# noir-lang/acvm

Hardware: AMD Instinct MI355X
Metric: witnesses solved/sec (whole node) (higher is better)
Workload: dtype u256 (8x u32 limbs, BN254-Fr Montgomery); 1 GPU; 10000-gate arithmetic-only ACIR, batch 2^20 witnesses over 1 GPU(s); opcodes=10000, global_batch=1048576, instances_per_gpu=1048576, tile_instances=131072, levels=41, not_solved_rank0_all_steps=68, algorithmic_bytes_per_witness=1025376, brillig_opcodes_inlined=0, parallelism=instances sharded x1, no collectives

## Files before the change

acvm_amd/__init__.py:

```python
import ctypes as C
import functools
import os

from . import acir

_HERE = os.path.dirname(os.path.abspath(__file__))
LIB_PATH = os.environ.get("ACVM_AMD_LIB") or os.path.join(_HERE, "libacvm_amd.so")

STATUS_SOLVED, STATUS_IN_PROGRESS, STATUS_FAILURE, STATUS_REQUIRES_FOREIGN_CALL = 0, 1, 2, 3
(ERR_NONE, ERR_MISSING_ASSIGNMENT, ERR_TOO_MANY_UNKNOWNS, ERR_UNSUPPORTED_BLACKBOX, ERR_UNSATISFIED, ERR_INDEX_OOB,
 ERR_BLACKBOX_FAILED, ERR_BRILLIG_FAILED, ERR_PANIC, ERR_DEVICE_LIMIT) = range(10)
LIMIT_BRILLIG_STEPS, LIMIT_BRILLIG_CALL_DEPTH, LIMIT_BRILLIG_MEMORY, LIMIT_DEVICE_MEMORY = 1, 2, 3, 4
ENC_BE32, ENC_LE32, ENC_MONT256_LE = 0, 1, 2
ENC_U8, ENC_U16, ENC_U32, ENC_U64, ENC_U128 = 16, 17, 18, 19, 20
LAYOUT_INSTANCE_MAJOR, LAYOUT_WITNESS_MAJOR = 0, 1
LAYOUT_BROADCAST = 16

ABI_SYMBOLS = [
    "acvm_last_error", "acvm_abi_version", "acvm_device_count", "acvm_set_device", "acvm_device_synchronize",
    "acvm_device_arch", "acvm_selftest", "acvm_debug_grumpkin", "acvm_debug_secp", "acvm_circuit_from_bytes", "acvm_circuit_free", "acvm_circuit_num_opcodes",
    "acvm_circuit_num_witnesses", "acvm_circuit_plan_stats", "acvm_batch_new", "acvm_batch_free", "acvm_batch_set_initial_witness",
    "acvm_batch_set_initial_witness_device", "acvm_batch_solve", "acvm_batch_solve_then_import", "acvm_batch_reset", "acvm_batch_set_instances", "acvm_batch_set_force_slow_path",
    "acvm_batch_results", "acvm_batch_witness", "acvm_batch_witness_map", "acvm_batch_stats",
    "acvm_batch_set_profiling", "acvm_batch_pending_foreign_call", "acvm_batch_pending_foreign_call_inputs",
    "acvm_batch_resolve_foreign_call", "acvm_circuit_assert_message", "acvm_circuit_witness_set", "acvm_batch_error_string",
    "acvm_batch_extract_witnesses", "acvm_batch_digest", "acvm_witness_map_decode", "acvm_witness_map_encode", "acvm_batch_witness_map_bytes",
    "acvm_device_malloc", "acvm_device_free", "acvm_device_upload", "acvm_batch_solve_opcode", "acvm_bb_stubbed", "acvm_bb_dummy",
    "acvm_new", "acvm_free", "acvm_solve", "acvm_solve_opcode", "acvm_get_status", "acvm_instruction_pointer", "acvm_witness_map", "acvm_finalize",
    "acvm_get_pending_foreign_call", "acvm_pending_foreign_call_inputs", "acvm_resolve_pending_foreign_call",
    "acvm_multi_new", "acvm_multi_free", "acvm_multi_num_groups", "acvm_multi_solve", "acvm_multi_results", "acvm_multi_num_witnesses",
    "acvm_multi_witness_map", "acvm_multi_locate", "acvm_debug_modmul_rate", "acvm_debug_secp_rate", "acvm_batch_new_ex", "acvm_circuit_plan_stats_ex",
    "acvm_tuning_set", "acvm_tuning_get", "acvm_tuning_key",
    "acvm_device_release_tables", "acvm_circuit_opcode_kinds", "acvm_batch_error_expression", "acvm_debug_stream_rate", "acvm_node_new", "acvm_node_free", "acvm_node_tile_instances", "acvm_node_num_devices", "acvm_node_solve", "acvm_node_stats",
    "acvm_debug_cpulist", "acvm_debug_device_locality", "acvm_debug_plan_fingerprint", "acvm_circuit_plans_built", "acvm_circuit_check_schedule", "acvm_batch_digest_blake2s",
    "acvm_batch_export_device", "acvm_device_download", "acvm_debug_fr", "acvm_debug_inverse_batch", "acvm_debug_inverse_batch_shared",
    "acvm_batch_import_device", "acvm_batch_solve_then_import_ex",
    "acvm_batch_import_device_parts", "acvm_debug_import_list_copies",
    "acvm_batch_import_device_masked", "acvm_batch_set_initial_witness_masked", "acvm_debug_import_missing",
    "acvm_debug_table_info", "acvm_debug_table_read", "acvm_debug_batch_tables",
    "acvm_batch_outcomes_device", "acvm_batch_export_device_list", "acvm_debug_export_h2d_bytes", "acvm_debug_select",
    "acvm_node_solve_device", "acvm_debug_node_io_bytes",
    "acvm_batch_foreign_call_sites", "acvm_batch_foreign_call_inputs_device", "acvm_batch_resolve_foreign_calls_device", "acvm_debug_foreign_call_stats",
    "acvm_batch_resolve_foreign_calls_device_rows",
    "acvm_node_set_foreign_call_handler", "acvm_node_foreign_stats",
    "acvm_batch_import_device_records", "acvm_batch_set_initial_witness_records", "acvm_node_solve_records",
    "acvm_batch_export_device_records", "acvm_batch_witness_records",
]


class AcvmError(RuntimeError):
    pass


class ExpressionHead(C.Structure):
    _fields_ = [("n_mul", C.c_uint32), ("n_lin", C.c_uint32), ("opcode_index", C.c_uint32), ("q_c", C.c_uint8 * 32)]


class ExportDesc(C.Structure):
    _fields_ = [("encoding", C.c_uint32), ("layout", C.c_uint32), ("first", C.c_uint32), ("n", C.c_uint32), ("witnesses", C.POINTER(C.c_uint32)),
                ("n_witnesses", C.c_uint32), ("stride", C.c_uint64)]


class OutcomesDesc(C.Structure):
    _fields_ = [("first", C.c_uint32), ("n", C.c_uint32), ("d_status", C.c_void_p), ("d_err", C.c_void_p), ("d_opcode_index", C.c_void_p),
                ("select_mask", C.c_uint32), ("d_selected", C.c_void_p)]


class ImportDesc(C.Structure):
    _fields_ = [("encoding", C.c_uint32), ("layout", C.c_uint32), ("columns", C.POINTER(C.c_uint32)), ("n_columns", C.c_uint32), ("stride", C.c_uint64)]


class ImportPart(C.Structure):
    _fields_ = [("d_values", C.c_void_p), ("encoding", C.c_uint32), ("layout", C.c_uint32), ("positions", C.POINTER(C.c_uint32)),
                ("columns", C.POINTER(C.c_uint32)), ("n", C.c_uint32), ("n_columns", C.c_uint32), ("stride", C.c_uint64)]


class RecordField(C.Structure):
    _fields_ = [("position", C.c_uint32), ("encoding", C.c_uint32), ("offset", C.c_uint64)]

# ... 297 lines not shown
    def as_dict(self):
        return {f: (list(getattr(self, f)) if f.startswith("class_") or f == "n_stream_launches" else getattr(self, f)) for f, _ in self._fields_}


_lib = None


def lib():
    global _lib
    if _lib is not None:
        return _lib
    if not os.path.exists(LIB_PATH):
        raise AcvmError(f"{LIB_PATH} is missing: build it with `python -m acvm_amd.build` (no CPU fallback exists)")
    L = C.CDLL(LIB_PATH)
    L.acvm_last_error.restype = C.c_char_p
    L.acvm_device_arch.argtypes = [C.c_char_p, C.c_size_t]
    L.acvm_selftest.argtypes = [C.c_uint32, C.c_uint64]
    L.acvm_debug_grumpkin.argtypes = [C.c_uint32, C.c_uint32, C.c_char_p, C.c_uint32, C.c_char_p]
    if hasattr(L, "acvm_debug_secp"):
        L.acvm_debug_secp.argtypes = [C.c_uint32, C.c_uint32, C.c_char_p, C.c_uint32, C.c_char_p]
    L.acvm_circuit_from_bytes.restype = C.c_void_p
    L.acvm_circuit_from_bytes.argtypes = [C.c_char_p, C.c_size_t]
    L.acvm_circuit_free.argtypes = [C.c_void_p]
    L.acvm_circuit_num_opcodes.restype = C.c_uint32
    L.acvm_circuit_num_opcodes.argtypes = [C.c_void_p]
    L.acvm_circuit_num_witnesses.restype = C.c_uint32
    L.acvm_circuit_num_witnesses.argtypes = [C.c_void_p]
    L.acvm_circuit_plan_stats.argtypes = [C.c_void_p, C.c_void_p, C.c_uint32, C.POINTER(Stats)]
    L.acvm_circuit_plan_stats_ex.argtypes = [C.c_void_p, C.c_void_p, C.c_uint32, C.c_uint32, C.c_void_p, C.c_uint32, C.POINTER(Stats)]
    L.acvm_debug_plan_fingerprint.argtypes = [C.c_void_p, C.c_void_p, C.c_uint32, C.c_uint32, C.c_void_p, C.c_uint32, C.POINTER(C.c_uint64), C.c_uint32]
    L.acvm_circuit_plans_built.restype = C.c_uint64
    L.acvm_circuit_plans_built.argtypes = [C.c_void_p]
    L.acvm_circuit_check_schedule.argtypes = [C.c_void_p, C.c_void_p, C.c_uint32, C.c_uint32, C.c_void_p, C.c_uint32, C.c_uint32, C.c_uint32, C.POINTER(C.c_uint64), C.c_char_p, C.c_size_t]
    L.acvm_batch_new.restype = C.c_void_p
    L.acvm_batch_new.argtypes = [C.c_void_p, C.c_void_p, C.c_uint32, C.c_void_p, C.c_uint32]
    L.acvm_batch_new_ex.restype = C.c_void_p
    L.acvm_batch_new_ex.argtypes = [C.c_void_p, C.c_void_p, C.c_uint32, C.c_void_p, C.c_uint32, C.c_uint32, C.c_void_p, C.c_uint32]
    L.acvm_batch_free.argtypes = [C.c_void_p]
    L.acvm_batch_set_initial_witness.argtypes = [C.c_void_p, C.c_void_p]
    L.acvm_batch_set_initial_witness_device.argtypes = [C.c_void_p, C.c_void_p]
    L.acvm_batch_solve.argtypes = [C.c_void_p]
    L.acvm_batch_solve_then_import.argtypes = [C.c_void_p, C.c_void_p]
    L.acvm_batch_reset.argtypes = [C.c_void_p]
    L.acvm_batch_set_instances.argtypes = [C.c_void_p, C.c_uint32]
    L.acvm_batch_set_force_slow_path.argtypes = [C.c_void_p, C.c_int]
    L.acvm_batch_set_profiling.argtypes = [C.c_void_p, C.c_int]
    L.acvm_batch_results.argtypes = [C.c_void_p, C.c_void_p]
    L.acvm_batch_witness.argtypes = [C.c_void_p, C.c_uint32, C.c_void_p, C.c_void_p]
    L.acvm_batch_witness_map.argtypes = [C.c_void_p, C.c_uint32, C.c_uint32, C.c_void_p, C.c_void_p]
    L.acvm_batch_stats.argtypes = [C.c_void_p, C.POINTER(Stats)]
    L.acvm_batch_pending_foreign_call.argtypes = [C.c_void_p, C.c_uint32, C.POINTER(ForeignCallInfo)]
    L.acvm_batch_pending_foreign_call_inputs.argtypes = [C.c_void_p, C.c_uint32, C.c_void_p, C.c_void_p]
    L.acvm_batch_resolve_foreign_call.argtypes = [C.c_void_p, C.c_uint32, C.c_uint32, C.c_char_p, C.c_void_p, C.c_char_p]
    L.acvm_circuit_assert_message.argtypes = [C.c_void_p, C.c_uint32, C.c_uint32, C.c_char_p, C.c_size_t]
    L.acvm_circuit_witness_set.argtypes = [C.c_void_p, C.c_int, C.c_void_p, C.c_uint32]
    L.acvm_batch_error_string.argtypes = [C.c_void_p, C.c_void_p, C.c_uint32, C.c_char_p, C.c_size_t]
    L.acvm_batch_extract_witnesses.argtypes = [C.c_void_p, C.c_void_p, C.c_uint32, C.c_uint32, C.c_uint32, C.c_void_p]
    L.acvm_batch_digest.argtypes = [C.c_void_p, C.c_uint32, C.c_uint32, C.c_void_p]
    L.acvm_batch_digest_blake2s.argtypes = [C.c_void_p, C.c_uint32, C.c_uint32, C.c_void_p]
    for f in (L.acvm_witness_map_decode, L.acvm_witness_map_encode, L.acvm_batch_witness_map_bytes):
        f.restype = C.c_longlong
    L.acvm_witness_map_decode.argtypes = [C.c_char_p, C.c_size_t, C.c_void_p, C.c_void_p, C.c_uint32]
    L.acvm_witness_map_encode.argtypes = [C.c_void_p, C.c_char_p, C.c_uint32, C.c_void_p, C.c_size_t]
    L.acvm_batch_witness_map_bytes.argtypes = [C.c_void_p, C.c_uint32, C.c_void_p, C.c_size_t]
    L.acvm_debug_modmul_rate.argtypes = [C.c_uint32, C.c_uint32, C.POINTER(C.c_double), C.POINTER(C.c_uint64)]
    if hasattr(L, "acvm_debug_fr"):
# ... 252 lines not shown
    _check(lib().acvm_debug_table_read(table, idx.ctypes.data, idx.size, out.ctypes.data))
    return out


SECP_PROBE_WORDS = ((2, 1), (1, 1), (2, 1), (2, 1), (1, 1), (1, 1), (3, 3), (5, 3), (1, 1), (2, 1), (2, 1), (1, 1),
                    (2, 1), (1, 1), (1, 4), (4, 3), (6, 2))


def debug_secp(curve, what, items):
    wi, wo = SECP_PROBE_WORDS[what]
    assert all(len(it) == wi for it in items)
    data = b"".join(int(v).to_bytes(32, "big") for it in items for v in it)
    out = C.create_string_buffer(32 * wo * max(len(items), 1))
    _check(lib().acvm_debug_secp(curve, what, data, len(items), out))
    raw = out.raw
    return [tuple(int.from_bytes(raw[32 * (wo * i + k):32 * (wo * i + k + 1)], "big") for k in range(wo)) for i in range(len(items))]


FR_PROBE_WORDS = ((16, 8), (16, 8), (8, 8), (16, 8), (16, 8), (8, 8), (8, 8), (8, 8), (8, 8), (8, 2), (8, 2), (1, 8), (8, 9), (9, 8), (18, 9), (18, 9), (9, 9),
                  (9, 1), (9, 9), (10, 9), (9, 9), (9, 9), (9, 9), (9, 9), (19, 9), (18, 9), (9, 9), (9, 1), (18, 9), (36, 9), (54, 9), (27, 9), (45, 9), (27, 9),
                  (45, 9), (18, 9), (36, 9), (27, 9))


def debug_fr(what, items, uniform=None):
    import numpy as np
    wi, wo = FR_PROBE_WORDS[what]
    a = np.ascontiguousarray(items, dtype=np.uint32).reshape(-1, wi)
    out = np.zeros((a.shape[0], wo), dtype=np.uint32)
    u = None if uniform is None else np.ascontiguousarray(uniform, dtype=np.uint32).reshape(18)
    _check(lib().acvm_debug_fr(what, a.ctypes.data, a.shape[0], None if u is None else u.ctypes.data, out.ctypes.data))
    return out


def debug_inverse_batch(den, inv_chunk, slot_of=None, inv_share=None):
    import numpy as np
    d = np.ascontiguousarray(den, dtype=np.uint32)
    n_jobs, B = d.shape[0], d.shape[1]
    assert d.shape == (n_jobs, B, 8)
    s = None if slot_of is None else np.ascontiguousarray(slot_of, dtype=np.uint32).reshape(n_jobs)
    inv, ev = np.zeros((n_jobs, B, 8), dtype=np.uint32), np.zeros(B, dtype=np.uint32)
    dc, hc = C.c_uint32(), C.c_uint32()
    if inv_share is None:
        _check(lib().acvm_debug_inverse_batch(d.ctypes.data, n_jobs, B, inv_chunk, None if s is None else s.ctypes.data, inv.ctypes.data, ev.ctypes.data,
                                              C.byref(dc), C.byref(hc)))
    else:
        _check(lib().acvm_debug_inverse_batch_shared(d.ctypes.data, n_jobs, B, inv_chunk, inv_share, None if s is None else s.ctypes.data, inv.ctypes.data,
                                                     ev.ctypes.data, C.byref(dc), C.byref(hc)))
    return inv, ev, dc.value, hc.value


def debug_select(status, select_mask, out=None, want_list=True):
    import numpy as np
    st = np.ascontiguousarray(status, dtype=np.uint8).reshape(-1)
    n = st.shape[0]
    lst = None
    if want_list:
        lst = np.zeros(n, dtype=np.uint32) if out is None else np.ascontiguousarray(out, dtype=np.uint32).reshape(n).copy()
    count = C.c_uint32()
    _check(lib().acvm_debug_select(st.ctypes.data if n else None, n, select_mask, lst.ctypes.data if lst is not None and n else None, C.byref(count)))
    return lst, count.value


def decompress_witness(data: bytes) -> dict:
    n = _check(lib().acvm_witness_map_decode(data, len(data), None, None, 0))
    ids = (C.c_uint32 * max(n, 1))()
    vals = C.create_string_buffer(32 * max(n, 1))
# ... 40 lines not shown
        n = lib().acvm_circuit_assert_message(self._h, acir_index, self.LOCATION_ACIR if brillig_index is None else brillig_index, buf, 4096)
        return None if n < 0 else buf.value.decode()

    def witness_set(self, which: str):
        n = _check(lib().acvm_circuit_witness_set(self._h, self.SETS[which], None, 0))
        arr = (C.c_uint32 * max(n, 1))()
        _check(lib().acvm_circuit_witness_set(self._h, self.SETS[which], arr, n))
        return list(arr[:n])

    def plan_stats(self, initial_ids, fold_digest=False, reuse_slots=False, keep=()) -> dict:
        ids = list(initial_ids)
        arr = (C.c_uint32 * max(len(ids), 1))(*ids)
        keep = list(keep)
        karr = (C.c_uint32 * max(len(keep), 1))(*keep)
        s = Stats()
        _check(lib().acvm_circuit_plan_stats_ex(self._h, arr, len(ids), (1 if fold_digest else 0) | (2 if reuse_slots else 0), karr, len(keep), C.byref(s)))
        return s.as_dict()

    def plans_built(self) -> int:
        return int(lib().acvm_circuit_plans_built(self._h))

    def check_schedule(self, initial_ids, n_instances=4096, fold_digest=False, reuse_slots=False, keep=(), host_solver=False, drop_wait=None) -> dict:
        ids = list(initial_ids)
        arr = (C.c_uint32 * max(len(ids), 1))(*ids)
        keep = list(keep)
        karr = (C.c_uint32 * max(len(keep), 1))(*keep)
        counts = (C.c_uint64 * 8)()
        text = C.create_string_buffer(1 << 14)
        rc = lib().acvm_circuit_check_schedule(self._h, arr, len(ids), (1 if fold_digest else 0) | (2 if reuse_slots else 0) | (0x100 if host_solver else 0),
                                               karr, len(keep), n_instances, 0xFFFFFFFF if drop_wait is None else drop_wait, counts, text, len(text))
        _check(rc)
        return {"ok": rc == 0, "n_launches": counts[0], "n_waits": counts[1], "n_accesses": counts[2], "n_records": counts[3], "n_findings": counts[4],
                "report": text.value.decode()}

    def plan_fingerprint(self, initial_ids, fold_digest=False, reuse_slots=False, keep=(), host_solver=False) -> list:
        ids = list(initial_ids)
        arr = (C.c_uint32 * max(len(ids), 1))(*ids)
        keep = list(keep)
        karr = (C.c_uint32 * max(len(keep), 1))(*keep)
        out = (C.c_uint64 * 128)()
        n = lib().acvm_debug_plan_fingerprint(self._h, arr, len(ids), (1 if fold_digest else 0) | (2 if reuse_slots else 0) | (0x100 if host_solver else 0),
                                              karr, len(keep), out, 128)
        _check(n)
        return list(out[:n])


class NodeOpts(C.Structure):
    _fields_ = [("n_devices", C.c_uint32), ("devices", C.POINTER(C.c_int)), ("tile_instances", C.c_uint32), ("batch_flags", C.c_uint32)]


class NodeStats(C.Structure):
    _fields_ = [("n_devices", C.c_uint32), ("tile_instances", C.c_uint32), ("n_instances", C.c_uint64), ("total_ms", C.c_double),
                ("device", C.c_int * 16), ("async_exact", C.c_uint32 * 16), ("tiles", C.c_uint32 * 16), ("exact_instances", C.c_uint32 * 16),
                ("lane_ms", C.c_double * 16), ("solve_device_ms", C.c_double * 16), ("h2d_wait_ms", C.c_double * 16), ("export_ms", C.c_double * 16),
                ("numa_node", C.c_int * 16), ("n_cpus_pinned", C.c_uint32 * 16), ("first_cpu", C.c_int * 16),
                ("plans_built", C.c_uint32), ("create_ms", C.c_double), ("plan_ms", C.c_double), ("host_rss_bytes", C.c_uint64)]


class Node:

    def __init__(self, circuit: "Circuit", initial_ids, keep=(), devices=None, tile=0, fold_digest=False, reuse_slots=False, solver: "BbSolver" = None):
        self.ids, self.keep = list(initial_ids), list(keep)
        self._solver = solver
        arr = (C.c_uint32 * max(len(self.ids), 1))(*self.ids)
        karr = (C.c_uint32 * max(len(self.keep), 1))(*self.keep)
        opts = NodeOpts()
# ... 620 lines not shown
```

acvm_amd/csrc/batch.cpp:

```cpp
#include <algorithm>
#include <chrono>
#include <cstdio>
#include <cstdlib>
#include <cstring>
#include <map>
#include <memory>
#include <new>
#include <stdexcept>
#include <string>
#include <vector>
#include "batch_internal.hpp"

static thread_local std::string g_last_error;
int set_err(int code, const std::string &msg) {
    g_last_error = msg;
    return code;
}

int stage_reserve(acvm_batch *b, size_t bytes) {
    if (bytes <= b->stage_cap) return 0;
    if (b->d_stage) { hipFree(b->d_stage); b->d_stage = nullptr; b->stage_cap = 0; }
    const size_t cap = std::max<size_t>(bytes + bytes / 4, (size_t)1 << 20);
    HIPCHK(hipMalloc((void **)&b->d_stage, cap));
    b->stage_cap = cap;
    return 0;
}
void clear_fc_store(acvm_batch *b) {
    for (auto &sl : b->fc_slots) {
        if (sl.device_owned) {
            sl.device_owned = false;
            sl.clear_pending = true;
            sl.bounds = FcBounds();
        }
        if (!sl.inst.empty()) { sl.inst.clear(); sl.dirty = true; }
    }
    b->fc_fail_msg.clear();
    b->fc_epoch++;
}

const char *acvm_last_error(void) { return g_last_error.c_str(); }
int acvm_abi_version(void) { return ACVM_AMD_ABI_VERSION; }

int acvm_device_count(void) {
    int n = 0;
// ... 141 lines not shown
    out->n_brillig_inlined = p.n_brillig_inlined;
    out->n_hash_chained = p.n_hash_chained;
    out->n_gate_out_asis = p.n_gate_out_mode[0];
    out->n_gate_out_weak = p.n_gate_out_mode[1];
    out->n_gate_out_canon = p.n_gate_out_mode[2];
    out->max_gate_bound = p.max_gate_bound;
    out->n_byte_planes = p.n_byte_planes;
    out->n_byte_plane_reads = p.n_byte_plane_reads;
    for (uint32_t L = 0; L + 1 < p.level_start.size(); L++) out->n_arith_launches += (p.level_start[L + 1] - p.level_start[L] + 65534) / 65535;
    for (int k = 0; k < 4; k++) out->class_algorithmic_bytes_per_instance[k] = p.cls_algorithmic_bytes[k];
    out->class_algorithmic_bytes_per_instance[CLS_GRUMPKIN] += p.cls_algorithmic_bytes[CLS_PEDERSEN] + p.cls_algorithmic_bytes[CLS_ECDSA] +
                                                               p.cls_algorithmic_bytes[CLS_HOSTBB];
}

int acvm_circuit_plan_stats(const acvm_circuit_t *c, const uint32_t *initial_ids, uint32_t n_initial, acvm_stats_t *out) {
    return acvm_circuit_plan_stats_ex(c, initial_ids, n_initial, 0, nullptr, 0, out);
}
int acvm_circuit_plan_stats_ex(const acvm_circuit_t *c, const uint32_t *initial_ids, uint32_t n_initial, uint32_t flags, const uint32_t *keep_ids,
                               uint32_t n_keep, acvm_stats_t *out) try {
    if (!c || !out || (n_initial && !initial_ids) || (n_keep && !keep_ids)) return set_err(ACVM_E_INVALID, "null argument");
    PlanOpts opts;
    opts.fold_digest = (flags & (ACVM_BATCH_FOLD_DIGEST | ACVM_BATCH_REUSE_SLOTS)) != 0;
    opts.reuse_slots = (flags & ACVM_BATCH_REUSE_SLOTS) != 0;
    opts.keep.assign(keep_ids, keep_ids + n_keep);
    const std::shared_ptr<const Plan> sp = plan_for(c, initial_ids, n_initial, opts);
    const Plan &p = *sp;
    plan_stats(p, out);
    if (!p.unsupported.empty()) return set_err(ACVM_E_UNSUPPORTED, p.unsupported);
    return 0;
} ABI_CATCH

static size_t plan_bytes(const Plan &p) {
    size_t words = p.gate_stream.size() + p.gate_offset.size() + p.prog.size() + p.prog_offset.size() + p.prog_scratch.size() + p.bytecode.size() + p.slot_of.size() + p.kbound.size() +
                   p.unscale_index.size() + p.scaled_ids.size() + p.producer.size() + p.byte_plane_of.size() + p.dyn_offset.size();
    for (int k = 0; k < (int)N_CLS; k++) words += 2 * p.cls_offset[k].size();
    return words * 4 + (p.constants.size() + p.unscale.size()) * sizeof(FrH);
}
static void remember_plan(const acvm_circuit *c, const std::shared_ptr<const Plan> &sp) {
    auto &v = c->recent_plans;
    v.erase(std::remove(v.begin(), v.end(), sp), v.end());
    v.push_back(sp);
    size_t total = 0;
    for (auto &q : v) total += plan_bytes(*q);
    while (v.size() > 1 && (v.size() > 8 || total > (1ull << 30))) { total -= plan_bytes(*v.front()); v.erase(v.begin()); }
}
std::shared_ptr<const Plan> plan_for(const acvm_circuit *c, const uint32_t *initial_ids, uint32_t n_initial, const PlanOpts &opts) {
    PlanKey key;
    key.ids.assign(initial_ids, initial_ids + n_initial);
    if (opts.reuse_slots) key.keep = opts.keep;
    key.host_blackbox = opts.host_blackbox;
    key.fold_digest = opts.fold_digest;
    key.reuse_slots = opts.reuse_slots;
    for (unsigned i = 0; const char *name = tuning_key(i); i++) {
        int64_t v = 0;
        tuning_get(name, &v);
        key.tuning.push_back(v);
    }
    {
        std::lock_guard<std::mutex> g(c->plan_mutex);
        for (auto it = c->plan_cache.begin(); it != c->plan_cache.end();) {
            std::shared_ptr<const Plan> sp = it->second.lock();
            if (!sp) { it = c->plan_cache.erase(it); continue; }
            if (it->first == key) { c->n_plans_shared++; remember_plan(c, sp); return sp; }
            ++it;
        }
    }
    std::shared_ptr<const Plan> sp = std::make_shared<const Plan>(build_plan(*c->c, initial_ids, n_initial, opts));
    std::lock_guard<std::mutex> g(c->plan_mutex);
    c->n_plans_built++;
    c->plan_cache.push_back({std::move(key), sp});
    remember_plan(c, sp);
    return sp;
}
uint64_t acvm_circuit_plans_built(const acvm_circuit_t *c) {
    if (!c) return 0;
    std::lock_guard<std::mutex> g(c->plan_mutex);
    return c->n_plans_built;
}

int acvm_circuit_check_schedule(const acvm_circuit_t *c, const uint32_t *initial_ids, uint32_t n_initial, uint32_t flags, const uint32_t *keep_ids, uint32_t n_keep,
                                uint32_t n_instances, uint32_t drop_wait, uint64_t *counts, char *report, size_t report_len) try {
    if (!c || (n_initial && !initial_ids) || (n_keep && !keep_ids)) return set_err(ACVM_E_INVALID, "null argument");
    PlanOpts opts;
    opts.fold_digest = (flags & (ACVM_BATCH_FOLD_DIGEST | ACVM_BATCH_REUSE_SLOTS)) != 0;
    opts.reuse_slots = (flags & ACVM_BATCH_REUSE_SLOTS) != 0;
    opts.host_blackbox = (flags & 0x100u) != 0;
    opts.keep.assign(keep_ids, keep_ids + n_keep);
    const std::shared_ptr<const Plan> sp = plan_for(c, initial_ids, n_initial, opts);
    if (!sp->unsupported.empty()) return set_err(ACVM_E_UNSUPPORTED, sp->unsupported);
    const LaunchLayout lay = layout_launches(*sp, ((uint64_t)n_instances + 63) / 64 * 64);
    const LevelSchedule sched = level_schedule(*sp, lay);
    const ScheduleReport rep = check_level_schedule(*sp, lay, sched, drop_wait);
    if (counts) { counts[0] = rep.n_launches; counts[1] = rep.n_waits; counts[2] = rep.n_accesses; counts[3] = rep.n_records; counts[4] = rep.n_findings; }
    if (report && report_len) snprintf(report, report_len, "%s", rep.text.c_str());
    return rep.ok ? 0 : 1;
} ABI_CATCH

int acvm_debug_plan_fingerprint(const acvm_circuit_t *c, const uint32_t *initial_ids, uint32_t n_initial, uint32_t flags, const uint32_t *keep_ids,
                                uint32_t n_keep, uint64_t *out, uint32_t cap) try {
    if (!c || !out || (n_initial && !initial_ids) || (n_keep && !keep_ids)) return set_err(ACVM_E_INVALID, "null argument");
    PlanOpts opts;
    opts.fold_digest = (flags & (ACVM_BATCH_FOLD_DIGEST | ACVM_BATCH_REUSE_SLOTS)) != 0;
    opts.reuse_slots = (flags & ACVM_BATCH_REUSE_SLOTS) != 0;
    opts.host_blackbox = (flags & 0x100u) != 0;
    opts.keep.assign(keep_ids, keep_ids + n_keep);
    const Plan p = build_plan(*c->c, initial_ids, n_initial, opts);
    if (!p.unsupported.empty()) return set_err(ACVM_E_UNSUPPORTED, p.unsupported);
    std::vector<uint64_t> fp;
    auto fnv = [](const void *data, size_t bytes, uint64_t h = 0xcbf29ce484222325ull) {
        const uint8_t *b = (const uint8_t *)data;
        for (size_t i = 0; i < bytes; i++) { h ^= b[i]; h *= 0x100000001b3ull; }
        return h;
    };
    auto vec = [&](const std::vector<uint32_t> &v) { fp.push_back(fnv(v.data(), v.size() * 4) ^ (uint64_t)v.size() << 40); };
    vec(p.gate_stream); vec(p.gate_offset); vec(p.level_start); vec(p.dyn_offset); vec(p.dyn_level_start); vec(p.level_needs_inverse);
    for (int q = 0; q < N_HEAVY_LANES; q++) { vec(p.level_needs_heavy[q]); vec(p.inv_needs_heavy[q]); vec(p.lane_needs_main[q]); for (int q2 = 0; q2 < N_HEAVY_LANES; q2++) vec(p.lane_needs_lane[q][q2]); }
    vec(p.prog); vec(p.prog_offset); vec(p.prog_scratch); vec(p.slot_of); vec(p.kbound); vec(p.scaled_ids); vec(p.unscale_index); vec(p.bytecode); vec(p.producer); vec(p.byte_plane_of);
    fp.push_back(fnv(p.constants.data(), p.constants.size() * sizeof(FrH)));
    fp.push_back(fnv(p.unscale.data(), p.unscale.size() * sizeof(FrH)));
    fp.push_back(fnv(p.prog_class.data(), p.prog_class.size()));
    for (int k = 0; k < (int)N_CLS; k++) {
        vec(p.cls_level_start[k]);
        std::vector<uint32_t> sorted;
        for (size_t L = 0; L + 1 < p.cls_level_start[k].size(); L++) {
            std::vector<std::pair<uint32_t, uint32_t>> lv;
            for (uint32_t r = p.cls_level_start[k][L]; r < p.cls_level_start[k][L + 1]; r++) lv.push_back({p.cls_offset[k][r], p.cls_scratch[k][r]});
            std::sort(lv.begin(), lv.end());
            for (auto &x : lv) { sorted.push_back(x.first); sorted.push_back(x.second); }
        }
        vec(sorted);
    }
    const uint32_t scal[] = {p.n_witnesses, p.n_opcodes, p.n_levels, p.n_slots, p.mem_cells, p.n_inverse_slots, p.n_digest_segments, p.truncated_at, p.n_byte_planes};
    fp.push_back(fnv(scal, sizeof scal));
    for (size_t i = 0; i < fp.size() && i < cap; i++) out[i] = fp[i];
    return (int)fp.size();
} ABI_CATCH


static int batch_init(acvm_batch *b) {
    HIPCHK(hipGetDevice(&b->device));
    hipDeviceProp_t prop;
    HIPCHK(hipGetDeviceProperties(&prop, b->device));
    if (strncmp(prop.gcnArchName, "gfx950", 6) != 0)
        return set_err(ACVM_E_DEVICE, std::string("device is ") + prop.gcnArchName + ", this library is built for gfx950 only");
    HIPCHK(hipStreamCreateWithFlags(&b->stream, hipStreamNonBlocking));
    HIPCHK(hipStreamCreateWithFlags(&b->stream_dyn, hipStreamNonBlocking));
    HIPCHK(hipStreamCreateWithFlags(&b->stream_heavy, hipStreamNonBlocking));
    HIPCHK(hipStreamCreateWithFlags(&b->stream_heavy2, hipStreamNonBlocking));
    HIPCHK(hipStreamCreateWithFlags(&b->stream_heavy3, hipStreamNonBlocking));
    HIPCHK(hipStreamCreateWithFlags(&b->stream_digest, hipStreamNonBlocking));
    HIPCHK(hipEventCreate(&b->ev_start));
    HIPCHK(hipEventCreate(&b->ev_end));
    const Plan &p = b->plan();
    size_t w_bytes = (size_t)(b->reuse() ? p.n_slots : p.n_witnesses) * 2 * b->Bp * sizeof(uint4);
    HIPCHK(hipMalloc((void **)&b->d_W, w_bytes ? w_bytes : 16));
    if (int rc = upload(&b->d_gate_stream, p.gate_stream)) return rc;
    if (int rc = upload(&b->d_gate_offset, p.gate_offset)) return rc;
    std::vector<uint32_t> consts(p.constants.size() * 8);
    for (size_t i = 0; i < p.constants.size(); i++) {
        const FrH d = frh::to_device_form(p.constants[i]);
        memcpy(&consts[8 * i], d.l, 32);
    }
    if (int rc = upload(&b->d_consts, consts)) return rc;
    if (!p.scaled_ids.empty()) {
        std::vector<uint32_t> uc(p.unscale.size() * 8);
        for (size_t i = 0; i < p.unscale.size(); i++) {
            const FrH d = frh::to_device_form(p.unscale[i]);
            memcpy(&uc[8 * i], d.l, 32);
        }
        if (int rc = upload(&b->d_unscale_consts, uc)) return rc;
        for (size_t i = 0; i < p.unscale.size(); i++) {
            uint64_t c[4];
            frh::to_canonical(p.unscale[i], c);
            memcpy(&uc[8 * i], c, 32);
        }
        if (int rc = upload(&b->d_unscale_plain, uc)) return rc;
        if (int rc = upload(&b->d_unscale_index, p.unscale_index)) return rc;
        if (int rc = upload(&b->d_scaled_ids, p.scaled_ids)) return rc;
    }
    if (int rc = upload(&b->d_prog, p.prog)) return rc;
    if (int rc = upload(&b->d_prog_offset, p.prog_offset)) return rc;
    if (int rc = upload(&b->d_bytecode, p.bytecode)) return rc;
    if (int rc = upload(&b->d_init_ids, p.initial_ids)) return rc;
    if (p.n_byte_planes) {
        b->plane_of_input.resize(p.initial_ids.size());
        for (size_t i = 0; i < p.initial_ids.size(); i++) b->plane_of_input[i] = p.byte_plane_of[p.initial_ids[i]];
        if (int rc = upload(&b->d_byte_plane_of, p.byte_plane_of)) return rc;
        if (int rc = upload(&b->d_byte_plane_of_input, b->plane_of_input)) return rc;
        HIPCHK(hipMalloc((void **)&b->d_byte_plane, (size_t)p.n_byte_planes * b->Bp * 4));
        HIPCHK(hipMemsetAsync(b->d_byte_plane, 0, (size_t)p.n_byte_planes * b->Bp * 4, b->stream));
// ... 192 lines not shown
```

acvm_amd/csrc/batch.hpp:

```cpp
#pragma once
#include "../../include/acvm_amd.h"
#include "foreign_plan.hpp"
#include "import_plan.hpp"
#include "kernels.hpp"
#include "plan.hpp"
#include "schedule.hpp"
#include <map>
#include <memory>
#include <mutex>
#include <string>
#include <vector>

using namespace acvm;

int set_err(int code, const std::string &msg);
#define HIPCHK(expr)                                                                                      \
    do {                                                                                                  \
        hipError_t _e = (expr);                                                                           \
        if (_e != hipSuccess)                                                                             \
            return set_err(ACVM_E_DEVICE, std::string(#expr) + ": " + hipGetErrorString(_e));             \
    } while (0)

#define ABI_CATCH                                                                                          \
    catch (const std::bad_alloc &) { return set_err(ACVM_E_NOMEM, "out of host memory"); }                 \
// ... 22 lines not shown
    uint8_t *d_digests = nullptr;
    uint64_t *h2d = nullptr;
};

struct PlanKey {
    std::vector<uint32_t> ids, keep;
    bool host_blackbox = false, fold_digest = false, reuse_slots = false;
    std::vector<int64_t> tuning;
    bool operator==(const PlanKey &o) const {
        return ids == o.ids && keep == o.keep && host_blackbox == o.host_blackbox && fold_digest == o.fold_digest && reuse_slots == o.reuse_slots && tuning == o.tuning;
    }
};
struct acvm_circuit {
    std::unique_ptr<Circuit> c;
    mutable std::mutex plan_mutex;
    mutable std::vector<std::pair<PlanKey, std::weak_ptr<const Plan>>> plan_cache;
    mutable std::vector<std::shared_ptr<const Plan>> recent_plans;
    mutable uint64_t n_plans_built = 0, n_plans_shared = 0;
};
std::shared_ptr<const Plan> plan_for(const acvm_circuit *c, const uint32_t *initial_ids, uint32_t n_initial, const acvm::PlanOpts &opts);

struct acvm_batch {
    std::shared_ptr<const Plan> plan_ref;
    const Plan &plan() const { return *plan_ref; }
    LaunchLayout layout;
    LevelSchedule schedule;
    uint32_t B = 0;
    uint32_t capacity = 0;
    uint64_t Bp = 0;
    int device = 0;
    hipStream_t stream = nullptr;
    uint4 *d_W = nullptr, *d_Mem = nullptr;
    uint32_t *d_gate_stream = nullptr, *d_gate_offset = nullptr, *d_consts = nullptr;
    uint32_t *d_prog = nullptr, *d_prog_offset = nullptr, *d_bytecode = nullptr, *d_init_ids = nullptr, *d_producer = nullptr;
    uint32_t *d_dyn_offset = nullptr, *d_slow_start = nullptr;
    uint8_t *d_prog_class = nullptr;
    uint32_t *d_cls_offset[N_CLS] = {nullptr, nullptr, nullptr, nullptr, nullptr, nullptr, nullptr};
    uint32_t *d_cls_scratch_off[N_CLS] = {nullptr, nullptr, nullptr, nullptr, nullptr, nullptr, nullptr};
    uint32_t *d_cls_scratch[N_CLS] = {nullptr, nullptr, nullptr, nullptr, nullptr, nullptr, nullptr};
    DeviceProgram dp{};
    uint32_t *d_event = nullptr;
    uint32_t *d_event_base = nullptr;
    uint32_t *h_flag_count = nullptr;
    bool events_fresh = false;
    std::vector<uint32_t> h_event;
    bool events_clean = false;
    std::vector<uint32_t> slow_ids, slow_start;
    std::vector<int32_t> slow_index;
    std::vector<SlowResult> slow_res;
    uint32_t *d_slow_ids = nullptr, *d_assigned = nullptr;
    SlowResult *d_slow_res = nullptr;
    uint32_t slow_cap = 0, n_words = 0;
    bool inputs_set = false, solved = false, force_slow = false, profiling = false;
    hipEvent_t ev_start = nullptr, ev_end = nullptr;
    std::vector<hipEvent_t> ev_pool;
    double solve_device_ms = 0, arith_kernel_ms = 0, dyn_kernel_ms = 0, slow_path_ms = 0;
    double cls_kernel_ms[N_CLS] = {0, 0, 0, 0, 0, 0, 0};
    hipStream_t stream_dyn = nullptr, stream_heavy = nullptr, stream_heavy2 = nullptr, stream_heavy3 = nullptr, stream_digest = nullptr;
    PlanOpts opts;
    uint4 *d_leaves = nullptr;
    uint32_t *d_fp_g = nullptr, *d_fp_gs = nullptr, *d_fp_h = nullptr, *d_fp_hgen = nullptr;
    DigestTables fp{};
    uint32_t *d_slot_of = nullptr;
    uint4 *d_Wx = nullptr, *d_Memx = nullptr;
    uint32_t *d_init_rows = nullptr, *d_ids_x = nullptr;
    uint32_t *d_byte_plane_of = nullptr, *d_byte_plane_of_input = nullptr, *d_byte_plane = nullptr;
// ... 73 lines not shown
    std::vector<FcSlot> fc_slots;
    FcStoreSlot *d_fc_store = nullptr;
    uint32_t *d_fc_pend_desc = nullptr;
    uint4 *d_fc_pend_vals = nullptr;
    uint32_t fc_pend_desc_words = 0, fc_pend_vals_cap = 0, fc_lanes_cap = 0;
    std::vector<uint32_t> h_pend_desc, h_pend_vals;
    bool pend_host_valid = false;
    uint64_t n_fc_h2d_bytes = 0, n_fc_d2h_bytes = 0;
    hipEvent_t ev_fc[2] = {nullptr, nullptr};
    uint64_t fc_epoch = 1, fc_rows_key[4] = {0, 0, 0, 0};
    std::vector<uint32_t> fc_rows_host;
    uint32_t *d_fc_rows = nullptr;
    size_t fc_rows_cap = 0;
    uint8_t *d_fc_mask = nullptr;
    size_t fc_mask_cap = 0;
    bool fc_rows_valid = false, fc_rows_longest_valid = false;
    uint32_t fc_rows_longest = 0;
    double fc_inputs_ms = 0, fc_append_ms = 0;
    uint8_t *d_stage = nullptr;
    size_t stage_cap = 0;
    uint8_t *d_fetch = nullptr;
    bool stepping = false;
    uint32_t *d_br_scratch = nullptr, *d_br_lane = nullptr;
    size_t br_scratch_bytes = 0;
    uint32_t br_lane_cap = 0;
    bool br_retry_active = false;
    uint32_t br_max_regs = 1;
    uint32_t n_brillig_retries = 0;

    ~acvm_batch() {
        hipSetDevice(device);
        for (void *p : {(void *)d_W, (void *)d_Mem, (void *)d_gate_stream, (void *)d_gate_offset, (void *)d_consts, (void *)d_prog,
                        (void *)d_prog_offset, (void *)d_bytecode, (void *)d_init_ids, (void *)d_producer, (void *)d_dyn_offset,
                        (void *)d_slow_start, (void *)d_event_base, (void *)d_slow_ids, (void *)d_assigned, (void *)d_slow_res})
            if (p) hipFree(p);
        if (h_flag_count) hipHostFree(h_flag_count);
        for (int k = 0; k < (int)N_CLS; k++)
            for (void *p : {(void *)d_cls_offset[k], (void *)d_cls_scratch_off[k], (void *)d_cls_scratch[k]})
                if (p) hipFree(p);
        for (auto e : ev_pool) hipEventDestroy(e);
        for (auto e : ev_sync) hipEventDestroy(e);
        for (auto e : ev_heavy) hipEventDestroy(e);
        if (stream_heavy) hipStreamDestroy(stream_heavy);
        if (stream_heavy2) hipStreamDestroy(stream_heavy2);
        if (stream_heavy3) hipStreamDestroy(stream_heavy3);
        if (stream_digest) hipStreamDestroy(stream_digest);
        if (d_prog_class) hipFree(d_prog_class);
        if (d_leaves) hipFree(d_leaves);
        for (void *p : {(void *)d_fp_g, (void *)d_fp_gs, (void *)d_fp_h, (void *)d_fp_hgen})
            if (p) hipFree(p);
        if (d_slot_of) hipFree(d_slot_of);
        for (void *p : {(void *)d_Wx, (void *)d_Memx, (void *)d_init_rows, (void *)d_ids_x, (void *)d_byte_plane_of, (void *)d_byte_plane_of_input, (void *)d_byte_plane})
            if (p) hipFree(p);
        if (d_inv) hipFree(d_inv);
        for (void *p : {(void *)d_unscale_index, (void *)d_unscale_consts, (void *)d_unscale_plain, (void *)d_scaled_ids, (void *)d_unscale_m256})
            if (p) hipFree(p);
        if (d_ped_seed) hipFree(d_ped_seed);
        if (d_stage) hipFree(d_stage);
        if (d_fetch) hipFree(d_fetch);
        if (d_import_lists) hipFree(d_import_lists);
        if (d_missing) hipFree(d_missing);
        if (d_mask_result) hipFree(d_mask_result);
        if (h_mask_result) hipHostFree(h_mask_result);
        if (d_lane_map) hipFree(d_lane_map);
        if (d_record_out_tables) hipFree(d_record_out_tables);
        for (uint8_t *q : d_sink)
            if (q) hipFree(q);
// ... 47 lines not shown
```

acvm_amd/csrc/batch_schedule.cpp:

```cpp
#include <algorithm>
#include <chrono>
#include <cstdio>
#include <cstdlib>
#include <cstring>
#include <map>
#include <memory>
#include <new>
#include <stdexcept>
#include <string>
#include <vector>
#include "batch_internal.hpp"

struct LaunchTimers {
    std::vector<std::pair<hipEvent_t, hipEvent_t>> reg_pairs, dyn_pairs, cls_pairs[N_CLS];
    size_t ev_used = 0;
};

static int enqueue_level_schedule(acvm_batch *b, LaunchTimers *tm) {
    const Plan &p = b->plan();
    auto next_event = [&]() -> hipEvent_t {
        if (tm->ev_used == b->ev_pool.size()) {
            hipEvent_t e;
            hipEventCreate(&e);
            b->ev_pool.push_back(e);
        }
        return b->ev_pool[tm->ev_used++];
    };
    const bool prof = tm != nullptr;
    hipStream_t streams[N_SCHED_STREAMS] = {b->stream, b->stream_dyn, b->stream_heavy, b->stream_heavy2, b->stream_heavy3, b->stream_digest};
    const uint32_t n_sync = 2 * p.n_levels + 1;
    auto event_of = [&](uint32_t id) { return id < n_sync ? b->ev_sync[id] : b->ev_heavy[id - n_sync]; };
    for (const SchedStep &st : b->schedule.steps) {
        hipStream_t s = streams[st.stream];
        if (st.kind == SK_RECORD) { HIPCHK(hipEventRecord(event_of(st.event), s)); continue; }
        if (st.kind == SK_WAIT) { HIPCHK(hipStreamWaitEvent(s, event_of(st.event), 0)); continue; }
        const int k = st.cls;
        const uint32_t *off = b->d_cls_offset[k] + st.first, *soff = b->d_cls_scratch_off[k] + 2 * (size_t)st.first;
        const bool timed = prof && st.op != SO_EVENT_RESET && st.op != SO_TRUNCATE;
        hipEvent_t e0 = nullptr, e1 = nullptr;
        if (timed) { e0 = next_event(); hipEventRecord(e0, s); }
        switch (st.op) {
        case SO_EVENT_RESET:
            if (!b->events_fresh) launch_event_reset(s, b->d_event, b->B);
            b->events_fresh = false;
            break;
        case SO_GATES:
            launch_arith_level(s, b->d_W, b->Bp, b->B, b->d_gate_stream, b->d_gate_offset + st.first, st.count, b->d_consts, b->d_event, b->d_inv);
            break;
        case SO_GATES_LIGHT:
            launch_arith_light_level(s, b->d_W, b->Bp, b->B, b->d_gate_stream, b->d_gate_offset + st.first, st.count, b->d_inv, b->dp,
                                     b->d_cls_offset[CLS_LIGHT] + st.first2, st.count2, b->d_event);
            break;
        case SO_LIGHT: launch_light_level(s, b->d_W, b->Bp, b->B, b->dp, off, st.count, b->d_event); break;
        case SO_LIGHT_SL: launch_light_sl_level(s, b->d_W, b->Bp, b->B, b->dp, off, st.count, b->d_event); break;
        case SO_HASH_COOP: launch_hash_coop_level(s, b->d_W, b->Bp, b->B, b->dp, off, st.count, b->d_event, st.lds_words); break;
        case SO_HASH: launch_hash_level(s, b->d_W, b->Bp, b->B, b->dp, off, soff, st.count, b->d_event, b->d_cls_scratch[k]); break;
        case SO_GRUMPKIN: launch_grumpkin_level(s, b->d_W, b->Bp, b->B, b->dp, off, soff, st.count, b->d_event, b->d_cls_scratch[k]); break;
        case SO_BRILLIG: launch_brillig_level(s, b->d_W, b->Bp, b->B, b->dp, off, soff, st.count, b->d_event, b->d_cls_scratch[k]); break;
        case SO_PEDERSEN: launch_pedersen_level(s, b->d_W, b->Bp, b->B, b->dp, off, st.count, b->d_event, soff, b->d_cls_scratch[k]); break;
        case SO_ECDSA: launch_ecdsa_level(s, b->d_W, b->Bp, b->B, b->dp, off, st.count, b->d_event); break;
        case SO_DIGEST: launch_digest_fold_level(s, b->d_W, b->Bp, b->B, b->dp, off, st.count, b->fp, b->d_leaves); break;
        case SO_HOSTBB:
            for (uint32_t r = 0; r < st.count; r++)
                if (int rc = run_host_blackbox(b, p.prog[p.cls_offset[k][st.first + r] + 1], false, 0)) return rc;
            break;
        case SO_INVERSE:
            launch_inverse_batch(s, b->d_W, b->d_inv, b->Bp, b->B, b->d_gate_stream, b->d_dyn_offset + st.first, st.count, b->d_event, (uint32_t)p.tune.inv_chunk,
                                 inverse_share_clamp(p.tune.inv_share));
            break;
        case SO_TRUNCATE: launch_event_truncate(s, b->d_event, b->B, p.truncated_at); break;
        }
        if (timed) {
            e1 = next_event();
            hipEventRecord(e1, s);
            (st.op == SO_GATES || st.op == SO_GATES_LIGHT ? tm->reg_pairs : st.op == SO_INVERSE ? tm->dyn_pairs : tm->cls_pairs[k]).push_back({e0, e1});
        }
        if (st.op == SO_GATES || st.op == SO_GATES_LIGHT) b->n_launches += (st.count + 65534) / 65535;
        else if (st.op != SO_EVENT_RESET && st.op != SO_TRUNCATE) b->n_launches++;
    }
    return 0;
}

static int ensure_level_events(acvm_batch *b) {
    const size_t n_levels = b->plan().n_levels;
// ... 203 lines not shown
```

acvm_amd/csrc/fr_device.hpp:

```cpp
#pragma once
#include <hip/hip_runtime.h>
#include <stdint.h>

#define FR_HD __host__ __device__

namespace acvm {

struct Fr {
    uint32_t v[8];
};

#define FR_P0 0xf0000001u
#define FR_P1 0x43e1f593u
#define FR_P2 0x79b97091u
#define FR_P3 0x2833e848u
#define FR_P4 0x8181585du
#define FR_P5 0xb85045b6u
#define FR_P6 0xe131a029u
#define FR_P7 0x30644e72u
#define FR_N0INV 0xefffffffu

FR_HD __forceinline__ uint32_t fr_p(int i) {
    constexpr uint32_t P[8] = {FR_P0, FR_P1, FR_P2, FR_P3, FR_P4, FR_P5, FR_P6, FR_P7};
    return P[i];
// ... 290 lines not shown
#pragma unroll
    for (int k = 0; k < 9; k++) {
#pragma unroll
        for (int t = 0; t < N; t++)
#pragma unroll
            for (int i = 0; i <= k; i++) acc += (uint64_t)a[t].v[i] * b[t].v[k - i];
#pragma unroll
        for (int i = 0; i < k; i++) acc += (uint64_t)m[i] * fr_p29(k - i);
        const uint32_t lo = (uint32_t)acc;
        m[k] = (((lo & 1u) << 28) - lo) & M;
        acc += ((uint64_t)m[k] << 28) + m[k];
        acc >>= 29;
    }
#pragma unroll
    for (int k = 9; k < 17; k++) {
#pragma unroll
        for (int t = 0; t < N; t++)
#pragma unroll
            for (int i = k - 8; i < 9; i++) acc += (uint64_t)a[t].v[i] * b[t].v[k - i];
#pragma unroll
        for (int i = k - 8; i < 9; i++) acc += (uint64_t)m[i] * fr_p29(k - i);
        if (ADD) acc += h->v[k - 9];
        r.v[k - 9] = (uint32_t)acc & M;
        acc >>= 29;
    }
    r.v[8] = (uint32_t)acc;
    if (ADD) r.v[8] += h->v[8];
    return r;
}
template <int N>
FR_HD __forceinline__ Fr29 fr29_dot(const Fr29 (&a)[N], const Fr29 (&b)[N]) { return fr29_dot_impl<N, false>(a, b, nullptr); }
template <int N>
FR_HD __forceinline__ Fr29 fr29_dot_add(const Fr29 (&a)[N], const Fr29 (&b)[N], const Fr29 &h) { return fr29_dot_impl<N, true>(a, b, &h); }

#if defined(__HIP_DEVICE_COMPILE__) && !defined(FR_NO_ASM_BLOCKS)
#define FR_ASM_BLOCKS 1
#include "fr_blocks.inc"
#endif
#ifdef FR_BLOCKS_ALL
#undef fr29_mul
FR_HD __forceinline__ Fr29 fr29_mul(const Fr29 &a, const Fr29 &b) {
#if FR_ASM_BLOCKS
    return fr29_mul_blk(a, b);
#else
    return fr29_mul_c(a, b);
#endif
}
#endif
FR_HD __forceinline__ Fr29 fr29_mul_b(const Fr29 &a, const Fr29 &b) {
#if FR_ASM_BLOCKS
    return fr29_mul_blk(a, b);
#else
    return fr29_mul(a, b);
#endif
}
template <int N, unsigned UB>
FR_HD __forceinline__ Fr29 fr29_dot_add_b(const Fr29 (&a)[N], const Fr29 (&b)[N], const Fr29 &h) {
    static_assert(N == 1 || N == 2, "generated forms");
#if FR_ASM_BLOCKS
    if constexpr (N == 1) {
        static_assert(UB <= 1u, "one product");
        if constexpr (UB == 1u) return fr29_dot1_add_blk_u(a[0], b[0], h);
        else return fr29_dot1_add_blk_v(a[0], b[0], h);
    } else {
        static_assert(UB == 0u || UB == 2u || UB == 3u, "a uniform first factor pairs with a uniform second one");
        if constexpr (UB == 0u) return fr29_dot2_add_blk_vv(a[0], b[0], a[1], b[1], h);
// ... 259 lines not shown
```

acvm_amd/csrc/gate_eval.hpp:

```cpp
#pragma once
#include "fr_device.hpp"
#include "gate_record.hpp"

namespace acvm {

FR_HD __forceinline__ void gate_h_room(Fr29 &h, uint32_t &hw, uint32_t weight) {
    if (hw + weight > GATE_H_MAX) {
        h = fr29_weak(fr29_norm(h));
        hw = GATE_H_AFTER_WEAK;
    }
    hw += weight;
}
FR_HD __forceinline__ void gate_h_sub(Fr29 &h, const Fr29 &x, uint32_t klog2) {
    if (klog2 <= 1) {
#pragma unroll
        for (int i = 0; i < 9; i++) h.v[i] += fr_kp29_sub(1, i) - x.v[i];
    } else if (klog2 == 2) {
#pragma unroll
        for (int i = 0; i < 9; i++) h.v[i] += fr_kp29_sub(2, i) - x.v[i];
    } else {
#pragma unroll
        for (int i = 0; i < 9; i++) h.v[i] += fr_kp29_sub(3, i) - x.v[i];
    }
}
FR_HD __forceinline__ Fr29 gate_coef29(GateWords t) {
    Fr c;
#pragma unroll
    for (int i = 0; i < 8; i++) c.v[i] = t[i];
    return fr29_from(c);
}

template <class L>
FR_HD __forceinline__ Fr29 gate_operand(const L &ld, uint32_t slot, const Fr29 &local) {
    if (slot == GATE_LOCAL) {
        Fr29 r = local;
#if defined(__HIP_DEVICE_COMPILE__)
#pragma unroll
        for (int k = 0; k < 9; k++) asm volatile("" : "+v"(r.v[k]));
#endif
        return r;
    }
    return ld.load(slot);
}
FR_HD __forceinline__ GateWords gate_mac_entry(GateWords t0, uint32_t np_mac, uint32_t k) {
    return k < np_mac ? t0 + 10 * k : t0 + 10 * np_mac + 9 * (k - np_mac);
}
template <class L>
FR_HD __forceinline__ Fr29 gate_mac_operand(const L &ld, GateWords c, bool product, const Fr29 &local) {
    if (product) return fr29_mul_b(gate_operand(ld, c[8], local), gate_operand(ld, c[9], local));
    return gate_operand(ld, c[8], local);
}

template <class L>
FR_HD __forceinline__ Fr29 gate_eval(const L &ld, GateWords g, const Fr29 &local) {
    const uint32_t w0 = g[0], w5 = g[5], qc = g[3], kind = w0 & 0xff;
    const uint32_t np_mac = (w0 >> 8) & 0xff, nl_mac = (w0 >> 16) & 0xff, n_mac = np_mac + nl_mac;
    const uint32_t np_pos = w5 & 0xff, np_neg = (w5 >> 8) & 0xff, nl_pos = (w5 >> 16) & 0xff, nl_neg = w5 >> 24;
    const uint32_t sub_k = (w0 >> GATE_SUBK_SHIFT) & 3u;
    Fr29 h;
    uint32_t hw = 0;
    if (qc == GATE_COEF_ZERO) {
#pragma unroll
        for (int i = 0; i < 9; i++) h.v[i] = 0;
    } else {
        h = gate_coef29(ld.constant(qc));
        hw = 16;
    }
    GateWords t0 = g + 6;
    GateWords tp = t0 + 10 * np_mac + 9 * nl_mac;
    GateWords t = tp + 2 * np_pos;
    for (uint32_t i = 0; i < np_neg; i++, t += 2) {
        const Fr29 x = fr29_mul_b(gate_operand(ld, t[0], local), gate_operand(ld, t[1], local));
        gate_h_room(h, hw, 33);
        gate_h_sub(h, x, 1);
    }
    for (uint32_t i = 0; i < nl_pos; i++, t += 1) {
        const Fr29 x = gate_operand(ld, t[0], local);
        gate_h_room(h, hw, 16);
        h = fr29_addl(h, x);
    }
    for (uint32_t i = 0; i < nl_neg; i++, t += 1) {
        const Fr29 x = gate_operand(ld, t[0], local);
        gate_h_room(h, hw, 33);
        gate_h_sub(h, x, sub_k);
    }
    uint32_t im = 0, ip = 0, n_red = 0;
    bool normalised = false;
#define GATE_AFTER_REDUCTION() do { normalised = true; if (++n_red == GATE_REDUCTIONS_PER_WEAK) { h = fr29_weak(h); n_red = 0; } } while (0)
    for (; ip < np_pos && im < n_mac; ip++, im++) {
        GateWords c = gate_mac_entry(t0, np_mac, im);
        const Fr29 l[2] = {gate_operand(ld, tp[2 * ip], local), gate_mac_operand(ld, c, im < np_mac, local)};
        const Fr29 m[2] = {gate_operand(ld, tp[2 * ip + 1], local), gate_coef29(c)};
        h = fr29_dot_add_b<2, 2u>(l, m, h);
        GATE_AFTER_REDUCTION();
    }
    for (; im < n_mac; im += 2) {
        GateWords c0 = gate_mac_entry(t0, np_mac, im);
        if (n_mac - im == 1) {
            const Fr29 l[1] = {gate_mac_operand(ld, c0, im < np_mac, local)}, m[1] = {gate_coef29(c0)};
            h = fr29_dot_add_b<1, 1u>(l, m, h);
        } else {
            GateWords c1 = gate_mac_entry(t0, np_mac, im + 1);
            const Fr29 l[2] = {gate_mac_operand(ld, c0, im < np_mac, local), gate_mac_operand(ld, c1, im + 1 < np_mac, local)};
            const Fr29 m[2] = {gate_coef29(c0), gate_coef29(c1)};
            h = fr29_dot_add_b<2, 3u>(l, m, h);
        }
        GATE_AFTER_REDUCTION();
    }
    for (; ip < np_pos; ip += 2) {
        if (np_pos - ip == 1) {
            const Fr29 l[1] = {gate_operand(ld, tp[2 * ip], local)}, m[1] = {gate_operand(ld, tp[2 * ip + 1], local)};
            h = fr29_dot_add_b<1, 0u>(l, m, h);
        } else {
            const Fr29 l[2] = {gate_operand(ld, tp[2 * ip], local), gate_operand(ld, tp[2 * ip + 2], local)};
            const Fr29 m[2] = {gate_operand(ld, tp[2 * ip + 1], local), gate_operand(ld, tp[2 * ip + 3], local)};
            h = fr29_dot_add_b<2, 0u>(l, m, h);
        }
        GATE_AFTER_REDUCTION();
    }
#undef GATE_AFTER_REDUCTION
    Fr29 acc = normalised ? h : fr29_norm(h);
    if (kind == 2) {
        if (w0 & GATE_PRESUM_WEAK) acc = fr29_weak(acc);
        acc = fr29_mul_b(acc, ld.load_inverse(g[4]));
    }
    const uint32_t mode = kind == 0 ? GATE_OUT_CANON : (w0 >> GATE_OUT_SHIFT) & 3u;
    if (mode != GATE_OUT_ASIS) {
        acc = fr29_weak(acc);
        if (mode == GATE_OUT_CANON) {
            if (ld.any(acc.v[8] >= fr_p29(8))) acc = fr29_csub(acc, 0);
        }
// ... 6 lines not shown
```

acvm_amd/csrc/gate_record.hpp:

```cpp
#pragma once
#include <stdint.h>

#if defined(__HIPCC__)
#define GATE_HD __host__ __device__
#else
#define GATE_HD
#endif

namespace acvm {

#if defined(__HIP_DEVICE_COMPILE__)
typedef const uint32_t __attribute__((address_space(4))) *GateWords;
#define GATE_WORDS(p) ((::acvm::GateWords)(uintptr_t)(p))
#else
typedef const uint32_t *GateWords;
#define GATE_WORDS(p) ((::acvm::GateWords)(p))
#endif

static constexpr uint32_t GATE_LOCAL = 0xFFFFFFFFu;
static constexpr uint32_t GATE_TAIL_FLAG = 1u << 24;
static constexpr uint32_t GATE_SETLOCAL_FLAG = 1u << 25;
static constexpr uint32_t GATE_OUT_SHIFT = 26;
static constexpr uint32_t GATE_OUT_ASIS = 0;
static constexpr uint32_t GATE_OUT_WEAK = 1;
static constexpr uint32_t GATE_OUT_CANON = 2;
static constexpr uint32_t GATE_SUBK_SHIFT = 28;
static constexpr uint32_t GATE_PRESUM_WEAK = 1u << 30;
static constexpr uint32_t GATE_COEF_ZERO = 0xFFFFFFFDu;

static constexpr uint32_t GATE_H_MAX = 111;
static constexpr uint32_t GATE_H_AFTER_WEAK = 17;
static constexpr uint32_t GATE_REDUCTIONS_PER_WEAK = 16;

static constexpr uint32_t GATE_K_CANON = 256, GATE_K_WEAK = 264, GATE_K_ROW_MAX = 1354, GATE_K_INVERSE = 359;
GATE_HD inline uint32_t gate_k_product(uint32_t ka, uint32_t kb) {
    return (uint32_t)(((uint64_t)ka * kb * 1549u + ((1ull << 26) - 1)) >> 26);
}

GATE_HD inline uint32_t gate_record_words(GateWords g) {
    const uint32_t w0 = g[0], w5 = g[5];
    return 6u + 10u * ((w0 >> 8) & 0xff) + 9u * ((w0 >> 16) & 0xff) + 2u * ((w5 & 0xff) + ((w5 >> 8) & 0xff)) + ((w5 >> 16) & 0xff) + (w5 >> 24);
}

}
```

acvm_amd/csrc/kernels.hip:

```cpp
#include "ops_common.hpp"
#include "fr_probe.hpp"
#include "inverse_batch.hpp"
#include "kernels.hpp"
#include "export_encode.hpp"
#include "export_source.hpp"
#include "tuning.hpp"

namespace acvm {

template <bool ALIGNED>
__global__ void __launch_bounds__(256) import_witness_kernel(uint4 *__restrict__ W, uint64_t Bp, uint32_t B,
                                                             const uint8_t *__restrict__ in, const uint32_t *__restrict__ ids,
                                                             uint32_t n_in, const uint32_t *__restrict__ gate, const uint32_t *__restrict__ plane_of_input,
                                                             uint32_t *__restrict__ plane, uint32_t *__restrict__ event_reset) {
    __shared__ uint4 tile[4][2][65];
    __shared__ uint32_t tile_low[4][64];
    if (gate && *gate != 0u) return;
    const uint32_t t = threadIdx.x;
    const uint64_t j0 = (uint64_t)blockIdx.x * 64u;
    const uint32_t k0 = blockIdx.y * 4u;
    {
        const uint32_t ji = t >> 2, kk = t & 3u;
        const uint64_t j = j0 + ji;
        const uint32_t k = k0 + kk;
// ... 231 lines not shown
    __syncthreads();
#pragma unroll
    for (uint32_t step = 0; step < export_tile_steps(T); step++) {
        const ExportTileUnit q = export_tile_unit(T, t, step);
        const uint64_t i = i0 + q.ji;
        const uint32_t k = kb + q.kk;
        if (i >= a.n || k >= a.n_sel) continue;
        const uint64_t at = export_element_index(EXPORT_INSTANCE_MAJOR, a.stride, i, k);
        export_store_nt(a.out + 2 * at + q.half, tile[q.kk][q.half][q.ji]);
        if (a.mask && q.half == 0) a.mask[at] = tile_assigned[q.kk][q.ji];
    }
}
__global__ void __launch_bounds__(256) unscale_slow_kernel(uint4 *__restrict__ W, uint64_t Bp, const uint32_t *__restrict__ slow_ids,
                                                           uint32_t n_slow, const uint32_t *__restrict__ scaled_ids, uint32_t n_scaled,
                                                           const uint32_t *__restrict__ consts, const uint32_t *__restrict__ producer,
                                                           const uint32_t *__restrict__ start_opcode) {
    const uint64_t i = (uint64_t)blockIdx.x * blockDim.x + threadIdx.x;
    if (i >= (uint64_t)n_slow * n_scaled) return;
    const uint32_t k = (uint32_t)(i / n_slow), t = (uint32_t)(i % n_slow);
    const uint64_t j = slow_ids[t];
    const uint32_t w = scaled_ids[k];
    if (producer[w] >= start_opcode[t]) return;
    fr_store(W, w, Bp, j, fr_mul(fr_load(W, w, Bp, j), fr_const(consts, k)));
}

#ifndef ARITH_BLOCK
#define ARITH_BLOCK 256
#endif
#ifndef ARITH_WAVES_MIN
#define ARITH_WAVES_MIN 6
#endif
__global__ void __launch_bounds__(ARITH_BLOCK) __attribute__((amdgpu_waves_per_eu(ARITH_WAVES_MIN, 8)))
arith_level_kernel(uint4 *__restrict__ W, uint64_t Bp, uint32_t B, const uint32_t *__restrict__ gate_stream, const uint32_t *__restrict__ gate_offset,
                   const uint32_t *__restrict__ consts, uint32_t *__restrict__ event, const uint4 *__restrict__ Inv) {
    arith_level_body(W, Bp, B, gate_stream, gate_offset, consts, event, Inv, blockIdx.y);
}

struct InverseDevicePolicy {
    static __device__ __forceinline__ Fr load_den(const uint4 *W, uint32_t row, uint64_t Bp, uint64_t j) { return fr_load(W, row, Bp, j); }
    static __device__ __forceinline__ Fr load_den_last(const uint4 *W, uint32_t row, uint64_t Bp, uint64_t j) { return fr_load_nt(W, row, Bp, j); }
    static __device__ __forceinline__ void park(uint4 *Inv, uint32_t slot, uint64_t Bp, uint64_t j, const Fr &a) { fr_store(Inv, slot, Bp, j, a); }
    static __device__ __forceinline__ Fr parked(const uint4 *Inv, uint32_t slot, uint64_t Bp, uint64_t j) { return fr_load(Inv, slot, Bp, j); }
    static __device__ __forceinline__ void store_inverse(uint4 *Inv, uint32_t slot, uint64_t Bp, uint64_t j, const Fr &a) { fr_store_nt(Inv, slot, Bp, j, a); }
    static __device__ __forceinline__ void flag(uint32_t *event, uint64_t j, uint32_t opcode) { flag_instance(event, j, opcode); }
};
__global__ void __launch_bounds__(64) inverse_batch_kernel(const uint4 *__restrict__ W, uint4 *__restrict__ Inv, uint64_t Bp, uint32_t B,
                                                           const uint32_t *__restrict__ gate_stream, const uint32_t *__restrict__ job_offset,
                                                           uint32_t n_jobs, uint32_t chunk, uint32_t *__restrict__ event) {
    const uint64_t j = (uint64_t)blockIdx.x * 64 + threadIdx.x;
    if (j >= B) return;
    const uint32_t first = blockIdx.y * chunk;
    const uint32_t n = n_jobs - first < chunk ? n_jobs - first : chunk;
    inverse_batch_body<InverseDevicePolicy>(W, Inv, Bp, j, gate_stream, job_offset, first, n, event);
}
template <int G>
__global__ void __launch_bounds__(64 * G) inverse_batch_kernel_shared(const uint4 *__restrict__ W, uint4 *__restrict__ Inv, uint64_t Bp, uint32_t B,
                                                                      const uint32_t *__restrict__ gate_stream, const uint32_t *__restrict__ job_offset,
                                                                      uint32_t n_jobs, uint32_t chunk, uint32_t *__restrict__ event) {
    __shared__ uint32_t rows[(G + 1) * INVERSE_SHARE_ROW_WORDS];
    const uint32_t lane = threadIdx.x & 63u, w = __builtin_amdgcn_readfirstlane(threadIdx.x >> 6);
    const uint64_t j = (uint64_t)blockIdx.x * (64 * G) + threadIdx.x;
    const bool live = j < B;
    const uint32_t first = blockIdx.y * chunk;
    const uint32_t n = n_jobs - first < chunk ? n_jobs - first : chunk;
    Fr29 total = fr29_from(fr_one());
    if (live) total = inverse_batch_forward<InverseDevicePolicy>(W, Inv, Bp, j, gate_stream, job_offset, first, n, event);
    inverse_share_row_store(rows, w, lane, total);
    __syncthreads();
// ... 78 lines not shown
        }
        auto same = [](const Fr29 &p, const Fr29 &q) {
            uint32_t d = 0;
#pragma unroll
            for (int k = 0; k < 9; k++) d |= p.v[k] ^ q.v[k];
            return d == 0;
        };
        if (!same(fr29_mul_b(x, y), fr29_mul(x, y)) || !same(fr29_mul_b(y, x), fr29_mul(y, x))) bad |= 512;
        const Fr29 l1[1] = {x}, m1v[1] = {y}, m1u[1] = {u};
        if (!same(fr29_dot_add_b<1, 0u>(l1, m1v, h), fr29_dot_add<1>(l1, m1v, h))) bad |= 1024;
        if (!same(fr29_dot_add_b<1, 1u>(l1, m1u, h), fr29_dot_add<1>(l1, m1u, h))) bad |= 1024;
        const Fr29 l2[2] = {x, z}, m2vv[2] = {y, x}, m2vu[2] = {y, u}, m2uu[2] = {w, u};
        if (!same(fr29_dot_add_b<2, 0u>(l2, m2vv, h), fr29_dot_add<2>(l2, m2vv, h))) bad |= 2048;
        if (!same(fr29_dot_add_b<2, 2u>(l2, m2vu, h), fr29_dot_add<2>(l2, m2vu, h))) bad |= 2048;
        if (!same(fr29_dot_add_b<2, 3u>(l2, m2uu, h), fr29_dot_add<2>(l2, m2uu, h))) bad |= 2048;
    }
    if (bad) atomicAdd(mismatches, 1u);
}

__global__ void __launch_bounds__(64) fr_probe_kernel(uint32_t what, const uint32_t *__restrict__ in, uint32_t n_items, uint32_t words_in, uint32_t words_out,
                                                      FrProbeUniform un, uint32_t *__restrict__ out) {
    const uint32_t t = blockIdx.x * 64 + threadIdx.x;
    if (t >= n_items) return;
    fr_probe_item(what, in + (size_t)t * words_in, un, out + (size_t)t * words_out);
}
uint32_t fr_probe_words(uint32_t what, bool out) { return out ? fr_probe_words_out(what) : fr_probe_words_in(what); }
void launch_fr_probe(hipStream_t s, uint32_t what, const uint32_t *in, uint32_t n_items, const uint32_t *uniform18, uint32_t *out) {
    if (!n_items || what >= FRP_COUNT) return;
    FrProbeUniform un;
    for (int k = 0; k < 18; k++) un.u[k / 9].v[k % 9] = uniform18 ? uniform18[k] : 0u;
    hipLaunchKernelGGL(fr_probe_kernel, dim3((n_items + 63) / 64), dim3(64), 0, s, what, in, n_items, fr_probe_words_in(what), fr_probe_words_out(what), un, out);
}

__global__ void __launch_bounds__(256) modmul_rate_kernel(uint32_t *__restrict__ out, uint32_t seed, uint32_t iters) {
    Fr29 a, b;
#pragma unroll
    for (int i = 0; i < 9; i++) {
        a.v[i] = ((threadIdx.x + 1) * 2654435761u + seed + i) & 0x1fffffffu;
        b.v[i] = (a.v[i] ^ 0x5bd1e995u) & 0x1fffffffu;
    }
    a.v[8] &= 0xfffffu;
    b.v[8] &= 0xfffffu;
    for (uint32_t i = 0; i < iters; i++) {
        a = fr29_mul(a, b);
        b = fr29_mul(b, a);
    }
    uint32_t s = 0;
#pragma unroll
    for (int i = 0; i < 9; i++) s += a.v[i] ^ b.v[i];
    out[(uint64_t)blockIdx.x * blockDim.x + threadIdx.x] = s;
}
__global__ void __launch_bounds__(256) stream_rate_kernel(const uint4 *__restrict__ a, const uint4 *__restrict__ b, uint4 *__restrict__ out) {
    const size_t i = (size_t)blockIdx.x * 256 + threadIdx.x;
    const uint4 x = a[i], y = b[i];
    out[i] = make_uint4(x.x ^ y.x, x.y ^ y.y, x.z ^ y.z, x.w ^ y.w);
}
void launch_stream_rate(hipStream_t s, const uint4 *a, const uint4 *b, uint4 *out, uint64_t n) {
    hipLaunchKernelGGL(stream_rate_kernel, dim3((unsigned)(n / 256)), dim3(256), 0, s, a, b, out);
}
void launch_modmul_rate(hipStream_t s, uint32_t *out, uint32_t blocks, uint32_t iters) {
    hipLaunchKernelGGL(modmul_rate_kernel, dim3(blocks), dim3(256), 0, s, out, 1u, iters);
}

__global__ void gather_initial_kernel(uint4 *__restrict__ Wx, uint64_t Bpx, const uint4 *__restrict__ W, uint64_t Bp, const uint32_t *__restrict__ init_ids,
                                      const uint32_t *__restrict__ init_rows, uint32_t n_init, const uint32_t *__restrict__ slow_ids, uint32_t n_slow) {
    const uint64_t i = (uint64_t)blockIdx.x * blockDim.x + threadIdx.x;
// ... 92 lines not shown
        hipLaunchKernelGGL(export_device_im_kernel<EXPORT_TILE_T>, dim3((x.n + EXPORT_TILE_I - 1u) / EXPORT_TILE_I, m), dim3(EXPORT_THREADS), 0, s, a, done * EXPORT_TILE_T);
    }
}
void launch_export_device_list(hipStream_t s, const ExportDevice &x, const uint4 *W, uint64_t Bp, const uint32_t *row_of, const uint32_t *producer, const Unscale &u,
                               const uint32_t *u_factor, const ExportListSource &src) {
    if (!x.n || !x.n_sel) return;
    const ExportArgs a{W, Bp, 0u, x.n, x.sel, x.n_sel, x.n_witnesses, row_of, producer, u.index, u_factor, x.encoding, x.stride, (uint4 *)x.out, x.mask};
    if (x.layout == EXPORT_WITNESS_MAJOR || x.n_sel < EXPORT_WAVES) {
        for_grid_y_chunks(x.n_sel, [&](uint32_t done, uint32_t m) { hipLaunchKernelGGL(export_list_direct_kernel, dim3((x.n + 255u) / 256u, m), dim3(256), 0, s, a, src, x.layout, done); });
        return;
    }
    const uint32_t tiles = (x.n_sel + EXPORT_TILE_T - 1u) / EXPORT_TILE_T;
    for_grid_y_chunks(tiles, [&](uint32_t done, uint32_t m) {
        hipLaunchKernelGGL(export_list_im_kernel<EXPORT_TILE_T>, dim3((x.n + EXPORT_TILE_I - 1u) / EXPORT_TILE_I, m), dim3(EXPORT_THREADS), 0, s, a, src, done * EXPORT_TILE_T);
    });
}
void launch_export_device_lanes(hipStream_t s, const ExportDevice &x, const uint4 *W, uint64_t Bp, bool side, const uint32_t *lanes, uint32_t n_lanes,
                                const uint32_t *assigned_bits, uint32_t n_slow) {
    if (!n_lanes || !x.n_sel) return;
    const ExportArgs a{W, Bp, x.first, x.n, x.sel, x.n_sel, x.n_witnesses, nullptr, nullptr, nullptr, nullptr, x.encoding, x.stride, (uint4 *)x.out, x.mask};
    for (uint32_t done = 0; done < x.n_sel; done += 65535u) {
        const uint32_t m = x.n_sel - done > 65535u ? 65535u : x.n_sel - done;
        hipLaunchKernelGGL(export_device_lanes_kernel, dim3((n_lanes + 255u) / 256u, m), dim3(256), 0, s, a, lanes, n_lanes, side, assigned_bits, n_slow, x.layout, done);
    }
}
void launch_unscale_slow(hipStream_t s, uint4 *W, uint64_t Bp, const uint32_t *slow_ids, uint32_t n_slow, const Unscale &u, const uint32_t *producer,
                         const uint32_t *start_opcode) {
    const uint64_t n = (uint64_t)n_slow * u.n_scaled;
    if (!n) return;
    hipLaunchKernelGGL(unscale_slow_kernel, dim3((unsigned)((n + 255) / 256)), dim3(256), 0, s, W, Bp, slow_ids, n_slow, u.scaled_ids, u.n_scaled,
                       u.consts, producer, start_opcode);
}
void launch_arith_level(hipStream_t s, uint4 *W, uint64_t Bp, uint32_t B, const uint32_t *gate_stream, const uint32_t *gate_offset,
                        uint32_t n_gates, const uint32_t *consts, uint32_t *event, const uint4 *inv) {
    for (uint32_t done = 0; done < n_gates;) {
        uint32_t n = n_gates - done > 65535u ? 65535u : n_gates - done;
        hipLaunchKernelGGL(arith_level_kernel, dim3((B + ARITH_BLOCK - 1) / ARITH_BLOCK, n), dim3(ARITH_BLOCK), 0, s, W, Bp, B, gate_stream, gate_offset + done, consts, event, inv);
        done += n;
    }
}
void launch_inverse_batch(hipStream_t s, const uint4 *W, uint4 *inv, uint64_t Bp, uint32_t B, const uint32_t *gate_stream,
                          const uint32_t *job_offset, uint32_t n_jobs, uint32_t *event, uint32_t inv_chunk, uint32_t inv_share) {
    if (!n_jobs || !B) return;
    const uint32_t G = inverse_share_clamp(inv_share), waves = (B + 63) / 64;
    const auto kernel = G == 8 ? inverse_batch_kernel_shared<8> : G == 4 ? inverse_batch_kernel_shared<4> : G == 2 ? inverse_batch_kernel_shared<2> : inverse_batch_kernel;
    const uint32_t cap = std::min<uint32_t>(std::max<uint32_t>(inv_chunk, 1), 65536), n_chunks = (n_jobs + cap - 1) / cap;
    const uint32_t chunk = (n_jobs + n_chunks - 1) / n_chunks;
    for (uint32_t done = 0; done < n_jobs;) {
        const uint32_t n = (uint32_t)std::min<uint64_t>(n_jobs - done, (uint64_t)chunk * 65535u);
        hipLaunchKernelGGL(kernel, dim3((waves + G - 1) / G, (n + chunk - 1) / chunk), dim3(64 * G), 0, s, W, inv, Bp, B, gate_stream, job_offset + done, n, chunk, event);
        done += n;
    }
}
void launch_fr_selftest(hipStream_t s, uint64_t seed, uint32_t n, uint32_t *mismatches) {
    if (!n) return;
    hipLaunchKernelGGL(fr_selftest_kernel, dim3((n + 255) / 256), dim3(256), 0, s, seed, n, mismatches);
}
__global__ void __launch_bounds__(256) event_reset_kernel(uint32_t *__restrict__ event, uint32_t B) {
    const uint32_t i = blockIdx.x * 256 + threadIdx.x;
    if (i < B) event[i] = 0xFFFFFFFFu;
    else if (i < B + 2) event[(int)(i - B) - 4] = 0u;
}
__global__ void __launch_bounds__(256) event_truncate_kernel(uint32_t *__restrict__ event, uint32_t B, uint32_t opcode) {
    const uint32_t i = blockIdx.x * 256 + threadIdx.x;
    if (i < B) event[i] = min(event[i], opcode);
    if (i == 0) event[-4] = B;
}
void launch_event_reset(hipStream_t s, uint32_t *event, uint32_t B) {
    hipLaunchKernelGGL(event_reset_kernel, dim3((B + 2) / 256 + 1), dim3(256), 0, s, event, B);
}
// ... 21 lines not shown
```

acvm_amd/csrc/kernels.hpp:

```cpp
#pragma once
#include "grumpkin_host.hpp"
#include <hip/hip_runtime.h>
#include <stdint.h>

namespace acvm {

struct SlowResult {
    uint32_t status, err, opcode_index, aux0, aux1;
    uint32_t msg, x0, x1;
    uint32_t n_call_stack;
    uint32_t call_stack[16];
    uint32_t val[8];
};

struct FcStoreSlot {
    const uint32_t *desc;
    const uint4 *vals;
};
struct FcLanes {
    uint32_t *pend_desc;
    uint32_t pend_desc_words;
    uint4 *pend_vals;
    uint32_t pend_vals_cap;
};
// ... 97 lines not shown
    const uint32_t *assigned_bits;
    uint32_t n_slow;
};
void launch_export_device_list(hipStream_t s, const ExportDevice &x, const uint4 *W, uint64_t Bp, const uint32_t *row_of, const uint32_t *producer, const Unscale &u,
                               const uint32_t *u_factor, const ExportListSource &src);
void launch_export_narrow_list(hipStream_t s, const ExportDevice &x, const uint4 *W, uint64_t Bp, const uint32_t *row_of, const uint32_t *producer, const Unscale &u,
                               const ExportListSource &src);
struct RecordExport {
    const uint4 *W;
    uint64_t Bp;
    uint32_t first, n;
    ExportListSource src;
    uint32_t n_witnesses;
    const uint32_t *row_of, *producer;
    const uint32_t *u_index, *u_plain, *u_m256;
    uint8_t *out;
    uint64_t pitch;
    const uint32_t *windows, *fields;
};
void launch_export_records(hipStream_t s, const RecordExport &x, uint32_t n_windows);
void launch_outcomes_fill(hipStream_t s, uint32_t n, uint8_t *status, uint8_t *err, uint32_t *opcode_index);
void launch_outcomes_lanes(hipStream_t s, const uint32_t *records, uint32_t n_lanes, uint32_t n, uint8_t *status, uint8_t *err, uint32_t *opcode_index);
void launch_lane_map_scatter(hipStream_t s, int32_t *lane_of, uint32_t n_instances, const uint32_t *ids, uint32_t n_slow);
void launch_scatter_rows32(hipStream_t s, const uint32_t *rows, const uint32_t *lanes, uint32_t n_lanes, uint32_t n, uint8_t *out);
size_t select_scratch_words(uint32_t n);
void launch_select(hipStream_t s, const uint8_t *status, uint32_t first, uint32_t n, uint32_t select_mask, uint32_t *scratch, uint32_t *out, uint32_t *count);
void launch_gather_initial(hipStream_t s, uint4 *Wx, uint64_t Bpx, const uint4 *W, uint64_t Bp, const uint32_t *init_ids, const uint32_t *init_rows, uint32_t n_init,
                           const uint32_t *slow_ids, uint32_t n_slow);
void launch_gather_columns(hipStream_t s, uint4 *Wx, uint64_t Bpx, const uint4 *W, uint64_t Bp, uint32_t n_rows, const uint32_t *slow_ids, uint32_t n_slow,
                           const uint32_t *unscale_index, const uint32_t *unscale_consts, const uint32_t *producer, const uint32_t *start_opcode);
void launch_unscale_slow(hipStream_t s, uint4 *W, uint64_t Bp, const uint32_t *slow_ids, uint32_t n_slow, const Unscale &u, const uint32_t *producer,
                         const uint32_t *start_opcode);
void launch_arith_level(hipStream_t s, uint4 *W, uint64_t Bp, uint32_t B, const uint32_t *gate_stream, const uint32_t *gate_offset,
                        uint32_t n_gates, const uint32_t *consts, uint32_t *event, const uint4 *inv);
void launch_inverse_batch(hipStream_t s, const uint4 *W, uint4 *inv, uint64_t Bp, uint32_t B, const uint32_t *gate_stream,
                          const uint32_t *job_offset, uint32_t n_jobs, uint32_t *event, uint32_t inv_chunk, uint32_t inv_share);
inline uint32_t inverse_share_clamp(int64_t v) { return v >= 8 ? 8u : v >= 4 ? 4u : v >= 2 ? 2u : 1u; }
void launch_arith_light_level(hipStream_t s, uint4 *W, uint64_t Bp, uint32_t B, const uint32_t *gate_stream, const uint32_t *gate_offset, uint32_t n_gates,
                              const uint4 *inv, const DeviceProgram &dp, const uint32_t *light_offsets, uint32_t n_light, uint32_t *event);
void launch_modmul_rate(hipStream_t s, uint32_t *out, uint32_t blocks, uint32_t iters);
void launch_secp_rate(hipStream_t s, uint32_t curve, uint32_t *out, uint32_t blocks, uint32_t iters);
void launch_stream_rate(hipStream_t s, const uint4 *a, const uint4 *b, uint4 *out, uint64_t n);
void launch_fr_selftest(hipStream_t s, uint64_t seed, uint32_t n, uint32_t *mismatches);
uint32_t fr_probe_words(uint32_t what, bool out);
void launch_fr_probe(hipStream_t s, uint32_t what, const uint32_t *in, uint32_t n_items, const uint32_t *uniform18, uint32_t *out);
void launch_fill_u32(hipStream_t s, uint32_t *p, uint32_t v, uint64_t n);
void launch_event_reset(hipStream_t s, uint32_t *event, uint32_t B);
void launch_event_truncate(hipStream_t s, uint32_t *event, uint32_t B, uint32_t opcode);
void launch_min_u32(hipStream_t s, uint32_t *p, uint32_t v, uint64_t n);
void launch_init_assigned(hipStream_t s, uint32_t *assigned, uint32_t n_slow, uint32_t n_words, uint32_t n_witnesses,
                          const uint32_t *producer, const uint32_t *start_opcode);

void launch_light_level(hipStream_t s, uint4 *W, uint64_t Bp, uint32_t B, const DeviceProgram &dp, const uint32_t *offsets, uint32_t n,
                        uint32_t *event);
void launch_light_sl_level(hipStream_t s, uint4 *W, uint64_t Bp, uint32_t B, const DeviceProgram &dp, const uint32_t *offsets, uint32_t n,
                           uint32_t *event);
void launch_hash_level(hipStream_t s, uint4 *W, uint64_t Bp, uint32_t B, const DeviceProgram &dp, const uint32_t *offsets,
                       const uint32_t *scratch_off, uint32_t n, uint32_t *event, uint32_t *scratch);
void launch_hash_coop_level(hipStream_t s, uint4 *W, uint64_t Bp, uint32_t B, const DeviceProgram &dp, const uint32_t *offsets, uint32_t n, uint32_t *event, uint32_t lds_words);
void launch_grumpkin_level(hipStream_t s, uint4 *W, uint64_t Bp, uint32_t B, const DeviceProgram &dp, const uint32_t *offsets,
                           const uint32_t *scratch_off, uint32_t n, uint32_t *event, uint32_t *scratch);
void launch_pedersen_seeds(hipStream_t s, const GrumpkinTables &T, const uint32_t *keys, uint32_t n, uint32_t *out);
void launch_pedersen_level(hipStream_t s, uint4 *W, uint64_t Bp, uint32_t B, const DeviceProgram &dp, const uint32_t *offsets, uint32_t n,
                           uint32_t *event, const uint32_t *scratch_off = nullptr, uint32_t *scratch = nullptr);
void launch_brillig_level(hipStream_t s, uint4 *W, uint64_t Bp, uint32_t B, const DeviceProgram &dp, const uint32_t *offsets,
                          const uint32_t *scratch_off, uint32_t n, uint32_t *event, uint32_t *scratch);

void launch_exact_init(hipStream_t s, const ExactLanes &L);
struct ExactScratch { uint32_t *hash, *grumpkin, *brillig; };
void launch_exact_run(hipStream_t s, uint4 *W, uint64_t Bp, const DeviceProgram &dp, const ExactLanes &L, uint32_t op_begin, uint32_t op_end, bool replay_memory,
                      const uint8_t *prog_class, const ExactScratch &sc);
void launch_grumpkin_probe(hipStream_t s, const GrumpkinTables &T, uint32_t what, uint32_t param, const uint32_t *in, uint32_t n_in, uint32_t *out);
void launch_table_gather(hipStream_t s, const uint4 *table, const uint64_t *entries, uint32_t n, uint4 *out);
void launch_secp_probe(hipStream_t s, uint32_t curve, uint32_t what, const uint32_t *in, uint32_t n_items, uint32_t words_in, uint32_t words_out, uint32_t *out,
                       const uint32_t *gtabs);
void launch_ecdsa_level(hipStream_t s, uint4 *W, uint64_t Bp, uint32_t B, const DeviceProgram &dp, const uint32_t *offsets, uint32_t n, uint32_t *event);
// ... 60 lines not shown
```

acvm_amd/csrc/kernels_ops.hip:

```cpp
#include "ops_kernel.hpp"
#include "ops_light.hpp"

namespace acvm {

struct LightOp {
    template <class P>
    static __device__ __forceinline__ OpResult run(const P &p, const uint32_t *__restrict__ rec, const DeviceProgram &dp, uint32_t *, SlowResult *, const ExactLanes *, uint32_t) {
        return dispatch_light(p, rec, dp.consts, dp.Mem);
    }
};
struct LightSlOp {
    template <class P>
    static __device__ __forceinline__ OpResult run(const P &p, const uint32_t *__restrict__ rec, const DeviceProgram &dp, uint32_t *, SlowResult *, const ExactLanes *, uint32_t) {
        __shared__ uint32_t regs[BRILLIG_SL_REGS * 8 * LIGHT_SL_BLOCK];
        return op_brillig_sl(p, rec, dp.consts, regs);
    }
};

__global__ void exact_init_kernel(ExactLanes L) {
    const uint32_t t = blockIdx.x * blockDim.x + threadIdx.x;
    if (t >= L.n_slow) return;
    SlowResult r;
    r.status = 1u;
    r.err = r.opcode_index = r.aux0 = r.aux1 = r.msg = r.x0 = r.x1 = r.n_call_stack = 0u;
// ... 78 lines not shown
    const uint32_t t = first + i;
    if (!active[t]) return;
    ExactPolicy p{W, Bp, L.slow_ids[t], L.assigned, L.n_slow, t};
    const OpResult r = hostbb_apply(p, func, rc[i], outs, n_out, vals + (uint64_t)i * n_out * 32);
    if (r.err) exact_fail(L, t, opcode, r);
}
void launch_hostbb_precheck(hipStream_t s, const ExactLanes &L, uint32_t opcode, const uint32_t *sel, uint32_t n_sel, uint8_t *active) {
    if (!L.n_slow) return;
    hipLaunchKernelGGL(hostbb_precheck_kernel, dim3((L.n_slow + 255) / 256), dim3(256), 0, s, L, opcode, sel, n_sel, active);
}
void launch_hostbb_gather(hipStream_t s, const uint4 *W, uint64_t Bp, const uint32_t *ids, uint32_t first, uint32_t n_lanes, const uint32_t *sel,
                          uint32_t n_sel, uint8_t *out, const uint32_t *slot_of) {
    if (!n_lanes || !n_sel) return;
    hipLaunchKernelGGL(hostbb_gather_kernel, dim3((n_lanes + 255) / 256, n_sel), dim3(256), 0, s, W, Bp, ids, first, n_lanes, sel, n_sel, out, slot_of);
}
void launch_hostbb_apply_level(hipStream_t s, uint4 *W, uint64_t Bp, uint32_t first, uint32_t n_lanes, uint32_t opcode, uint32_t func, const uint32_t *outs,
                               uint32_t n_out, const uint8_t *rc, const uint8_t *vals, uint32_t *event, const uint32_t *slot_of) {
    if (!n_lanes) return;
    hipLaunchKernelGGL(hostbb_apply_level_kernel, dim3((n_lanes + 255) / 256), dim3(256), 0, s, W, Bp, first, n_lanes, opcode, func, outs, n_out, rc, vals, event, slot_of);
}
void launch_hostbb_apply_exact(hipStream_t s, uint4 *W, uint64_t Bp, const ExactLanes &L, uint32_t first, uint32_t n_lanes, uint32_t opcode, uint32_t func,
                               const uint32_t *outs, uint32_t n_out, const uint8_t *active, const uint8_t *rc, const uint8_t *vals) {
    if (!n_lanes) return;
    hipLaunchKernelGGL(hostbb_apply_exact_kernel, dim3((n_lanes + 63) / 64), dim3(64), 0, s, W, Bp, L, first, n_lanes, opcode, func, outs, n_out, active, rc, vals);
}

void launch_light_level(hipStream_t s, uint4 *W, uint64_t Bp, uint32_t B, const DeviceProgram &dp, const uint32_t *offsets, uint32_t n,
                        uint32_t *event) {
    launch_record_level<LightOp, 256>(s, W, Bp, B, dp, offsets, nullptr, n, event, nullptr);
}
__global__ void __launch_bounds__(256) __attribute__((amdgpu_waves_per_eu(6, 8)))
arith_light_level_kernel(uint4 *__restrict__ W, uint64_t Bp, uint32_t B, const uint32_t *__restrict__ gate_stream, const uint32_t *__restrict__ gate_offset,
                         const uint32_t *__restrict__ consts, uint32_t *__restrict__ event, const uint4 *__restrict__ Inv, uint32_t n_light,
                         const uint32_t *__restrict__ light_offsets, const uint32_t *__restrict__ prog, const uint32_t *__restrict__ slot_of, uint4 *Mem) {
    if (blockIdx.y >= n_light) {
        arith_level_body(W, Bp, B, gate_stream, gate_offset, consts, event, Inv, blockIdx.y - n_light);
        return;
    }
    const uint64_t j = (uint64_t)blockIdx.x * 256 + threadIdx.x;
    if (j >= B) return;
    const uint32_t *__restrict__ rec = prog + light_offsets[blockIdx.y];
    FastPolicy p{W, Bp, j, slot_of};
    const OpResult r = dispatch_light(p, rec, consts, Mem);
    if (r.err) flag_instance(event, j, rec[0] == K_RANGE_MULTI ? r.aux0 : rec[1]);
}
void launch_arith_light_level(hipStream_t s, uint4 *W, uint64_t Bp, uint32_t B, const uint32_t *gate_stream, const uint32_t *gate_offset, uint32_t n_gates,
                              const uint4 *inv, const DeviceProgram &dp, const uint32_t *light_offsets, uint32_t n_light, uint32_t *event) {
    if (!B || !(n_gates + n_light)) return;
    hipLaunchKernelGGL(arith_light_level_kernel, dim3((B + 255) / 256, n_gates + n_light), dim3(256), 0, s, W, Bp, B, gate_stream, gate_offset, dp.consts, event, inv,
                       n_light, light_offsets, dp.prog, dp.slot_of, dp.Mem);
}
void launch_light_sl_level(hipStream_t s, uint4 *W, uint64_t Bp, uint32_t B, const DeviceProgram &dp, const uint32_t *offsets, uint32_t n,
                           uint32_t *event) {
    launch_record_level<LightSlOp, LIGHT_SL_BLOCK>(s, W, Bp, B, dp, offsets, nullptr, n, event, nullptr);
}
void launch_exact_init(hipStream_t s, const ExactLanes &L) {
    if (!L.n_slow) return;
    hipLaunchKernelGGL(exact_init_kernel, dim3((L.n_slow + 255) / 256), dim3(256), 0, s, L);
}
void launch_exact_finish(hipStream_t s, const ExactLanes &L, uint32_t min_ip) {
    if (!L.n_slow) return;
    hipLaunchKernelGGL(exact_finish_kernel, dim3((L.n_slow + 255) / 256), dim3(256), 0, s, L, min_ip);
}

}
```

acvm_amd/csrc/ops_common.hpp:

```cpp
#pragma once
#include "fr_device.hpp"
#include "gate_eval.hpp"

namespace acvm {

static constexpr uint32_t K_COEF_ONE = 0xFFFFFFFFu;
static constexpr uint32_t K_COEF_MINUS_ONE = 0xFFFFFFFEu;
static constexpr uint32_t K_COEF_ZERO = 0xFFFFFFFDu;
static constexpr uint32_t K_NONE = 0xFFFFFFFFu;

enum RecKind : uint32_t {
    K_ARITH = 0, K_RANGE = 1, K_LOGIC = 2, K_HASH = 3, K_PEDERSEN = 4, K_FIXED_BASE = 5, K_SCHNORR = 6, K_ZERO_OUT = 7,
    K_QUOTIENT = 8, K_TO_LE_RADIX = 9, K_MEM_INIT = 10, K_MEM_OP = 11, K_BRILLIG = 12, K_ECDSA = 13, K_PERM_SORT = 14,
    K_DIGEST_LEAF = 15, K_RANGE_MULTI = 16, K_BRILLIG_SL = 17
};

enum DevErr : uint32_t {
    DE_NONE = 0, DE_MISSING_ASSIGNMENT = 1, DE_TOO_MANY_UNKNOWNS = 2, DE_UNSUPPORTED_BLACKBOX = 3, DE_UNSATISFIED = 4,
    DE_INDEX_OOB = 5, DE_BLACKBOX_FAILED = 6, DE_BRILLIG_FAILED = 7, DE_PANIC = 8,
    DE_WAIT_FOREIGN_CALL = 100
};
enum DevMsg : uint32_t {
    DM_NONE = 0, DM_TWO_MUL_TERMS = 1, DM_LOGIC_BITS = 2, DM_FETCH_BYTES = 3, DM_HASH_OUTPUTS = 4, DM_KECCAK_VAR_LEN = 5,
    DM_MEM_INDEX_U64 = 6, DM_MEM_READ_EXPR = 7, DM_RADIX = 8, DM_LIMB_LOW = 9, DM_LIMB_HIGH = 10, DM_SCALAR = 11,
// ... 10 lines not shown
__device__ __forceinline__ OpResult op_fail(uint32_t e, uint32_t a0 = 0, uint32_t a1 = 0) { return OpResult{e, a0, a1, 0u, 0u, 0u}; }
__device__ __forceinline__ OpResult op_fail_msg(uint32_t e, uint32_t a0, uint32_t msg, uint32_t x0 = 0, uint32_t x1 = 0) {
    return OpResult{e, a0, 0u, msg, x0, x1};
}

__device__ __forceinline__ Fr apply_coef(const Fr &x, uint32_t coef, const uint32_t *__restrict__ consts) {
    if (coef == K_COEF_ONE) return x;
    if (coef == K_COEF_MINUS_ONE) return fr_neg(x);
    return fr_mul(x, fr_const(consts, coef));
}
__device__ __forceinline__ Fr apply_coef_prod(const Fr &a, const Fr &b, uint32_t coef, const uint32_t *__restrict__ consts) {
    const Fr29 t = fr29_mul(fr29_from(a), fr29_from(b));
    if (coef == K_COEF_ONE) return fr29_pack(fr29_cond_sub_p(t));
    if (coef == K_COEF_MINUS_ONE) return fr_neg(fr29_pack(fr29_cond_sub_p(t)));
    return fr29_pack(fr29_cond_sub_p(fr29_mul(t, fr29_from(fr_const(consts, coef)))));
}
static constexpr int EVENT_HDR_WORDS = 4;
__device__ __forceinline__ void flag_instance(uint32_t *__restrict__ event, uint64_t j, uint32_t opcode) {
    const bool first = atomicMin(&event[j], opcode) == 0xFFFFFFFFu;
    const uint64_t firsts = __builtin_amdgcn_ballot_w64(first);
    const uint32_t lane = __builtin_amdgcn_mbcnt_hi(~0u, __builtin_amdgcn_mbcnt_lo(~0u, 0u));
    if (first && (uint32_t)__builtin_ctzll(firsts) == lane) {
        const uint32_t n = (uint32_t)__builtin_popcountll(firsts);
        atomicAdd(event - 4, n);
        uint32_t *host = *(uint32_t *const *)(event - 2);
        if (host) __hip_atomic_fetch_add(host, n, __ATOMIC_RELAXED, __HIP_MEMORY_SCOPE_SYSTEM);
    }
}
struct GateDeviceLoader {
    const uint4 *__restrict__ W;
    const uint4 *__restrict__ Inv;
    const uint32_t *__restrict__ consts;
    uint64_t Bp, j;
    __device__ __forceinline__ Fr29 load(uint32_t slot) const {
#ifdef GATE_EXP_NO_LOADS
        Fr29 r;
#pragma unroll
        for (int i = 0; i < 9; i++) r.v[i] = ((uint32_t)j * 2654435761u + slot * 40503u + i) & 0x1fffffffu;
        r.v[8] &= 0xffffffu;
        return r;
#else
        return fr29_from(fr_load_nt(W, slot, Bp, j));
#endif
    }
    __device__ __forceinline__ Fr29 load_inverse(uint32_t slot) const { return fr29_from(fr_load_nt(Inv, slot, Bp, j)); }
    __device__ __forceinline__ GateWords constant(uint32_t idx) const { return GATE_WORDS(consts) + (uint64_t)idx * 8; }
    __device__ __forceinline__ bool any(bool x) const { return __builtin_amdgcn_ballot_w64(x) != 0; }
};
__device__ __forceinline__ void arith_level_body(uint4 *__restrict__ W, uint64_t Bp, uint32_t B, const uint32_t *__restrict__ gate_stream,
                                                 const uint32_t *__restrict__ gate_offset, const uint32_t *__restrict__ consts,
                                                 uint32_t *__restrict__ event, const uint4 *__restrict__ Inv, uint32_t gate_index) {
    const uint64_t j = (uint64_t)blockIdx.x * blockDim.x + threadIdx.x;
    if (j >= B) return;
    GateWords g = GATE_WORDS(gate_stream) + gate_offset[gate_index];
    const GateDeviceLoader ld{W, Inv, consts, Bp, j};
    Fr29 local = fr29_from(fr_zero());
    bool host = true;
    for (;;) {
        const uint32_t w0 = g[0], kind = w0 & 0xff, opcode = g[1], out = g[2];
        const Fr29 acc = gate_eval(ld, g, local);
        if (kind == 0) {
            uint32_t z = 0;
#pragma unroll
            for (int i = 0; i < 9; i++) z |= acc.v[i];
            if (z) flag_instance(event, j, opcode);
        } else {
#ifdef GATE_EXP_NO_STORES
            if (fr29_pack(acc).v[3] == 0x12345678u && acc.v[5] == 77u) event[j] = 0;
#else
            fr_store_nt(W, out, Bp, j, fr29_pack(acc));
#endif
        }
        if (!(w0 & GATE_TAIL_FLAG)) break;
        if (host || (w0 & GATE_SETLOCAL_FLAG)) local = acc;
        host = false;
        g += gate_record_words(g);
    }
}
__device__ __forceinline__ Fr coef_value(uint32_t coef, const uint32_t *__restrict__ consts) {
    if (coef == K_COEF_ONE) return fr_one();
    if (coef == K_COEF_MINUS_ONE) return fr_neg(fr_one());
    if (coef == K_COEF_ZERO) return fr_zero();
    return fr_const(consts, coef);
}
__device__ __forceinline__ Fr fr_r2() {
    Fr r = {{0x45b69bd4u, 0x38c2e14bu, 0x85883377u, 0x0ffedb18u, 0xabc6e54du, 0x7840f9f0u, 0x848b0f05u, 0x0a054a3eu}};
    return r;
}
// ... 161 lines not shown
```

acvm_amd/csrc/plan.cpp:

```cpp
#include "plan.hpp"
#include "gate_record.hpp"
#include "tuning.hpp"
#include "scratch_layout.hpp"
#include <algorithm>
#include <array>
#include <chrono>
#include <cstdlib>
#include <map>
#include <queue>
#include <stdexcept>
#include <unordered_map>

namespace acvm {
namespace {

struct ConstPool {
    std::vector<FrH> &pool;
    static constexpr uint32_t NONE = 0xFFFFFFFFu;
    struct Entry {
        FrH v, ninv;
        uint32_t id = NONE, inv_id = NONE;
        uint8_t has_inv = 0;
    };
    std::vector<Entry> ents;
    std::vector<uint64_t> slots;
    size_t mask = 0;
    FrH one = frh::one(), minus_one = frh::neg(frh::one());
    explicit ConstPool(std::vector<FrH> &p) : pool(p) { rehash(1u << 12); }
    static uint64_t hash(const FrH &c) {
        uint64_t h = c.l[0] * 0x9E3779B97F4A7C15ULL ^ c.l[1] * 0xC2B2AE3D27D4EB4FULL ^ c.l[2] * 0x165667B19E3779F9ULL ^ c.l[3] * 0x27D4EB2F165667C5ULL;
        h ^= h >> 29;
        h *= 0xBF58476D1CE4E5B9ULL;
        return h ^ h >> 32;
    }
// ... 224 lines not shown

void order_level_records(Plan &p) {
    const std::vector<uint32_t> &pg = p.prog;
    for (size_t L = 0; L < p.n_levels; L++) {
        {
            const int k = CLS_HASH;
            const uint32_t lo = p.cls_level_start[k][L], hi = p.cls_level_start[k][L + 1];
            std::vector<std::pair<uint32_t, uint32_t>> recs;
            for (int pass = 0; pass < 3 && hi > lo; pass++)
                for (uint32_t r = lo; r < hi; r++)
                    if (hash_launch_group(pg, p.cls_offset[k][r]) == pass) recs.push_back({p.cls_offset[k][r], p.cls_scratch[k][r]});
            for (uint32_t r = lo; r < hi; r++) { p.cls_offset[k][r] = recs[r - lo].first; p.cls_scratch[k][r] = recs[r - lo].second; }
        }
        {
            const int k = CLS_GRUMPKIN;
            const uint32_t lo = p.cls_level_start[k][L], hi = p.cls_level_start[k][L + 1];
            if (hi - lo > 1) {
                std::vector<std::pair<uint32_t, uint32_t>> recs;
                for (uint32_t r = lo; r < hi; r++) recs.push_back({p.cls_offset[k][r], p.cls_scratch[k][r]});
                std::stable_sort(recs.begin(), recs.end(), [&](const std::pair<uint32_t, uint32_t> &x, const std::pair<uint32_t, uint32_t> &y) {
                    auto rank = [&](uint32_t off) { const uint32_t kind = pg[off]; return kind == PK_SCHNORR ? 0 : kind == PK_PEDERSEN ? 1 : 2; };
                    return rank(x.first) < rank(y.first);
                });
                for (uint32_t r = lo; r < hi; r++) { p.cls_offset[k][r] = recs[r - lo].first; p.cls_scratch[k][r] = recs[r - lo].second; }
            }
        }
        for (const int k : {(int)CLS_LIGHT, (int)CLS_BRILLIG}) {
            const uint32_t lo = p.cls_level_start[k][L], hi = p.cls_level_start[k][L + 1];
            std::vector<std::pair<uint32_t, uint32_t>> recs;
            for (int pass = 0; pass < 2 && hi > lo; pass++)
                for (uint32_t r = lo; r < hi; r++)
                    if ((pg[p.cls_offset[k][r]] == PK_BRILLIG_SL) == (pass == 1)) recs.push_back({p.cls_offset[k][r], p.cls_scratch[k][r]});
            for (uint32_t r = lo; r < hi; r++) { p.cls_offset[k][r] = recs[r - lo].first; p.cls_scratch[k][r] = recs[r - lo].second; }
        }
    }
}

struct Block { uint32_t base = 0, cap = 0, len = 0, readable = 0, level = 0, rlevel = 0; bool seen = false; };
inline bool is_heavy(uint32_t cls) { return cls == CLS_HASH || cls == CLS_GRUMPKIN || cls == CLS_BRILLIG || cls == CLS_PEDERSEN || cls == CLS_ECDSA || cls == CLS_DIGEST; }

struct Planner {
    const Circuit &c;
    const uint32_t *initial_ids;
    const uint32_t n_initial;
    const PlanOpts &opts;
    const bool host_blackbox;
    const Tuning tune;
    const std::chrono::steady_clock::time_point t0 = std::chrono::steady_clock::now();
    Plan p;
    uint32_t nw = 0;
    std::vector<uint8_t> known;
    std::vector<uint32_t> level;
    ConstPool pool;
    std::map<uint32_t, Block> blocks;
    std::vector<std::vector<std::pair<uint32_t, uint32_t>>> out_slots;
    std::vector<uint32_t> sl_prog;
    std::unordered_map<uint32_t, std::pair<uint32_t, uint32_t>> sl_of;
    uint32_t sl_base = 0;
    std::vector<PendingGate> gates;
    std::vector<PendingRecord> records;
    std::vector<PendingInverse> inverses;
    std::vector<uint32_t> heavy_level;
    std::vector<uint8_t> wlane;
    std::vector<uint32_t> hlevel;
    uint32_t K_heavy = 1, D_heavy = 0, D_pedersen = 0, K_pedersen = 1;
    std::vector<std::pair<uint32_t, uint32_t>> heavy_reads;
// ... 1412 lines not shown
    }
};

}

Plan build_plan(const Circuit &c, const uint32_t *initial_ids, uint32_t n_initial, const PlanOpts &opts) {
    Planner b(c, initial_ids, n_initial, opts);
    b.p.tune = b.tune;
    b.p.n_opcodes = (uint32_t)c.opcodes.size();
    const bool v = b.tune.plan_validate != 0;
    if (!b.init()) return b.finish();
    if (!b.emit_in_order_program()) return b.finish();
    if (v) b.check_in_order_program();
    b.pin_witnesses();
    b.replay();
    if (v) b.check_replay();
    b.fuse_gate_pairs();
    if (v) b.check_pairs();
    b.assign_inverse_slots();
    if (v) b.check_inverse_slots();
    b.fold_digest_leaves();
    if (v) b.check_digest_leaves();
    b.fuse_range_checks();
    b.chain_hashes();
    b.merge_range_records();
    if (v) b.check_range_accounting();
    b.order_and_dependencies();
    if (v) b.check_dependencies();
    if (!b.assign_rows()) return b.finish();
    if (v) b.check_rows();
    b.lay_out();
    if (v) b.check_layout();
    order_level_records(b.p);
    return b.finish();
}

}
```

acvm_amd/csrc/plan.hpp:

```cpp
#pragma once
#include "circuit.hpp"
#include "tuning.hpp"
#include <algorithm>
#include <map>
#include <string>
#include <utility>
#include <vector>

namespace acvm {

static constexpr uint32_t COEF_ONE = 0xFFFFFFFFu;
static constexpr uint32_t COEF_MINUS_ONE = 0xFFFFFFFEu;
static constexpr uint32_t COEF_ZERO = 0xFFFFFFFDu;

enum GateKind : uint32_t { GATE_ASSERT = 0, GATE_SOLVE = 1, GATE_SOLVE_DYN = 2 };

static constexpr uint32_t GATE_HDR_WORDS = 5;

static constexpr uint32_t PLAN_HASH_COOP_FLAG = 0x100u;
static constexpr uint32_t PLAN_HASH_CHAIN_FLAG = 0x400u;
static constexpr uint32_t PLAN_HASH_RANGE_FLAG = 0x200u;
static constexpr uint32_t PLAN_HASH_COOP_MAX_BYTES = 1024;
enum ProgKind : uint32_t {
    PK_ARITH = 0, PK_RANGE = 1, PK_LOGIC = 2, PK_HASH = 3, PK_PEDERSEN = 4, PK_FIXED_BASE = 5, PK_SCHNORR = 6, PK_ZERO_OUT = 7,
    PK_QUOTIENT = 8, PK_TO_LE_RADIX = 9, PK_MEM_INIT = 10, PK_MEM_OP = 11, PK_BRILLIG = 12, PK_ECDSA = 13, PK_PERM_SORT = 14, PK_DIGEST_LEAF = 15, PK_RANGE_MULTI = 16, PK_BRILLIG_SL = 17
};
enum OpClass : uint32_t { CLS_LIGHT = 0, CLS_HASH = 1, CLS_GRUMPKIN = 2, CLS_BRILLIG = 3, CLS_PEDERSEN = 4, CLS_HOSTBB = 5, CLS_ECDSA = 6, CLS_DIGEST = 7, N_CLS = 8 };

struct Plan {
    Tuning tune;
    uint32_t n_witnesses = 0;
    uint32_t n_opcodes = 0;
    std::vector<uint32_t> initial_ids;
    std::vector<uint32_t> byte_plane_of;
    uint32_t n_byte_planes = 0, n_byte_plane_reads = 0;
    std::vector<uint32_t> gate_stream;
    std::vector<uint32_t> gate_offset;
    std::vector<uint32_t> level_start;
    std::vector<uint32_t> dyn_offset;
    std::vector<uint32_t> dyn_level_start;
    std::vector<uint32_t> level_needs_inverse;
    std::vector<uint32_t> level_needs_heavy[4];
    std::vector<uint32_t> inv_needs_heavy[4];
    std::vector<uint32_t> lane_needs_lane[4][4];
    std::vector<uint32_t> lane_needs_main[4];
    std::vector<FrH> constants;
    std::vector<uint32_t> scaled_ids;
    std::vector<FrH> unscale;
    std::vector<uint32_t> unscale_index;
    std::vector<uint32_t> kbound;
    uint32_t n_gate_out_mode[3] = {0, 0, 0};
    uint32_t max_gate_bound = 0;
    std::vector<uint32_t> prog;
    std::vector<uint32_t> prog_offset;
    std::vector<uint8_t> prog_class;
    std::vector<uint32_t> prog_scratch;
    std::vector<uint32_t> cls_offset[N_CLS];
    std::vector<uint32_t> cls_scratch[N_CLS];
    std::vector<uint32_t> cls_level_start[N_CLS];
    uint32_t n_levels = 0;
    uint32_t n_digest_segments = 0;
    std::vector<uint32_t> slot_of;
    uint32_t n_slots = 0;
    uint32_t mem_cells = 0;
    std::vector<uint32_t> bytecode;
    std::vector<uint32_t> producer;
    uint32_t truncated_at = 0xFFFFFFFFu;
    uint32_t n_fast_gates = 0, n_dyn_gates = 0, max_level_width = 0, n_other_records = 0;
    uint32_t n_gate_pairs = 0;
    uint32_t n_brillig_inlined = 0;
// ... 53 lines not shown
```

acvm_amd/csrc/probes.cpp:

```cpp
#include <algorithm>
#include <chrono>
#include <cstdio>
#include <cstdlib>
#include <cstring>
#include <map>
#include <memory>
#include <new>
#include <stdexcept>
#include <string>
#include <vector>
#include "batch_internal.hpp"

int acvm_selftest(uint32_t n, uint64_t seed) {
    uint32_t *d = nullptr, h = 0;
    HIPCHK(hipMalloc((void **)&d, 4));
    HIPCHK(hipMemset(d, 0, 4));
    launch_fr_selftest(nullptr, seed, n, d);
    HIPCHK(hipGetLastError());
    HIPCHK(hipDeviceSynchronize());
    HIPCHK(hipMemcpy(&h, d, 4, hipMemcpyDeviceToHost));
    hipFree(d);
    return (int)h;
}

static int product_rate(uint32_t field, uint32_t iters, uint32_t waves_per_simd, double *per_s, uint64_t *n_products) {
    if (!per_s || !iters || !waves_per_simd || field > 2) return set_err(ACVM_E_INVALID, "bad argument");
    int dev = 0;
    HIPCHK(hipGetDevice(&dev));
    hipDeviceProp_t prop;
    HIPCHK(hipGetDeviceProperties(&prop, dev));
    const uint32_t blocks = (uint32_t)prop.multiProcessorCount * waves_per_simd;
    uint32_t *d = nullptr;
    HIPCHK(hipMalloc((void **)&d, (size_t)blocks * 256 * 4));
    hipEvent_t e0, e1;
    HIPCHK(hipEventCreate(&e0));
    HIPCHK(hipEventCreate(&e1));
    float best = 1e30f;
    for (int r = 0; r < 4; r++) {
        hipEventRecord(e0, nullptr);
        if (field == 0) launch_modmul_rate(nullptr, d, blocks, iters);
        else launch_secp_rate(nullptr, field - 1, d, blocks, iters);
        hipEventRecord(e1, nullptr);
        hipEventSynchronize(e1);
        float ms = 0;
// ... 186 lines not shown
} ABI_CATCH

int acvm_debug_batch_tables(const acvm_batch_t *b, uint32_t *mask) {
    if (!b || !mask) return set_err(ACVM_E_INVALID, "null argument");
    const GrumpkinTables &t = b->dp.grumpkin;
    *mask = (t.ped2 && !t.pedw ? 1u : 0u) | (t.win16 ? 2u : 0u) | (t.pedw ? 4u : 0u) | (b->dp.ecdsa_g ? 8u : 0u);
    return 0;
}

int acvm_debug_fr(uint32_t what, const uint32_t *in, uint32_t n_items, const uint32_t *uniform18, uint32_t *out) try {
    const uint32_t wi = fr_probe_words(what, false), wo = fr_probe_words(what, true);
    if (!wi || !wo) return set_err(ACVM_E_INVALID, "no such routine");
    if (!n_items) return 0;
    if (!in || !out) return set_err(ACVM_E_INVALID, "null argument");
    uint32_t *d_in = nullptr, *d_out = nullptr;
    HIPCHK(hipMalloc((void **)&d_in, (size_t)n_items * wi * 4));
    if (hipMalloc((void **)&d_out, (size_t)n_items * wo * 4) != hipSuccess) {
        hipFree(d_in);
        return set_err(ACVM_E_DEVICE, "hipMalloc failed");
    }
    int rc = 0;
    auto step = [&](hipError_t e, const char *what_) { if (!rc && e != hipSuccess) rc = set_err(ACVM_E_DEVICE, std::string(what_) + ": " + hipGetErrorString(e)); };
    step(hipMemcpy(d_in, in, (size_t)n_items * wi * 4, hipMemcpyHostToDevice), "hipMemcpy");
    step(hipMemset(d_out, 0, (size_t)n_items * wo * 4), "hipMemset");
    if (!rc) launch_fr_probe(nullptr, what, d_in, n_items, uniform18, d_out);
    step(hipGetLastError(), "fr_probe_kernel");
    step(hipDeviceSynchronize(), "hipDeviceSynchronize");
    step(hipMemcpy(out, d_out, (size_t)n_items * wo * 4, hipMemcpyDeviceToHost), "hipMemcpy");
    hipFree(d_in);
    hipFree(d_out);
    return rc;
} ABI_CATCH

static int debug_inverse_batch(const uint32_t *den, uint32_t n_jobs, uint32_t B, uint32_t inv_chunk, uint32_t inv_share, const uint32_t *slot_of, uint32_t *inv_out,
                               uint32_t *event_out, uint32_t *device_count, uint32_t *host_count) {
    if (!den || !n_jobs || !B || !inv_out || !event_out || !device_count || !host_count) return set_err(ACVM_E_INVALID, "bad argument");
    if (slot_of) {
        std::vector<uint8_t> seen(n_jobs, 0);
        for (uint32_t k = 0; k < n_jobs; k++) {
            if (slot_of[k] >= n_jobs || seen[slot_of[k]]) return set_err(ACVM_E_INVALID, "slot_of is not a permutation");
            seen[slot_of[k]] = 1;
        }
    }
    const uint64_t Bp = ((uint64_t)B + 63) / 64 * 64;
    const size_t row = (size_t)2 * Bp, table_bytes = (size_t)n_jobs * row * sizeof(uint4);
    std::vector<uint4> hW((size_t)n_jobs * row, make_uint4(0, 0, 0, 0));
    std::vector<uint32_t> stream((size_t)n_jobs * 3), offset(n_jobs);
    for (uint32_t k = 0; k < n_jobs; k++) {
        for (uint32_t j = 0; j < B; j++) {
            const uint32_t *v = den + ((size_t)k * B + j) * 8;
            hW[(size_t)k * row + j] = make_uint4(v[0], v[1], v[2], v[3]);
            hW[(size_t)k * row + Bp + j] = make_uint4(v[4], v[5], v[6], v[7]);
        }
        stream[3 * (size_t)k] = k;
        stream[3 * (size_t)k + 1] = k;
        stream[3 * (size_t)k + 2] = slot_of ? slot_of[k] : k;
        offset[k] = 3 * k;
    }
    struct Mem {
        uint4 *W = nullptr, *inv = nullptr;
        uint32_t *stream = nullptr, *offset = nullptr, *event_base = nullptr, *event = nullptr, *h_count = nullptr;
        ~Mem() {
            for (void *p : {(void *)W, (void *)inv, (void *)stream, (void *)offset, (void *)event_base})
                if (p) hipFree(p);
            if (h_count) hipHostFree(h_count);
        }
// ... 60 lines not shown
```

acvm_amd/csrc/schedule_check.cpp:

```cpp
#include "gate_record.hpp"
#include "schedule.hpp"
#include <array>
#include <cstdio>
#include <string>

namespace acvm {
namespace {

constexpr uint32_t NONE = 0xFFFFFFFFu;
enum ResKind : int { RK_W = 0, RK_INV, RK_MEM, RK_BYTE_PLANE, RK_LEAF, RK_SCRATCH, N_RK };
const char *RES_NAME[N_RK] = {"witness row", "inverse row", "memory cell", "byte plane", "digest leaf", "class scratch"};
constexpr uint32_t K_WEAK_DOMAIN = 169u * 256u;

struct Res {
    int32_t w_launch = -1;
    uint32_t w_prog = 0;
    uint32_t tag = NONE;
    uint32_t kb = GATE_K_CANON;
    uint8_t canon = 1;
    uint8_t r_multi = 0;
    int32_t r_launch[N_SCHED_STREAMS] = {-1, -1, -1, -1, -1, -1};
    uint32_t r_prog[N_SCHED_STREAMS] = {0, 0, 0, 0, 0, 0};
};
struct Launch {
    uint8_t stream, op;
    uint32_t level, seq, step;
    std::array<uint32_t, N_SCHED_STREAMS> clock;
};

struct Checker {
    const Plan &p;
    const LaunchLayout &lay;
    const LevelSchedule &sch;
// ... 306 lines not shown
                if (!r->canon) c.finding("REPRESENTATION: " + std::string(who) + " reads witness " + std::to_string(w) + " (row " + std::to_string(row) + ") as it is in " + c.launch_name(c.cur) + " but its writer " + c.launch_name(r->w_launch) + " stored a relaxed row");
                if (c.p.unscale_index[w] != NONE) c.finding("REPRESENTATION: " + std::string(who) + " reads witness " + std::to_string(w) + " as it is in " + c.launch_name(c.cur) + " but the witness is stored scaled");
            }
            return r;
        }
        void rd(uint32_t w) override { row_read(w, true); }
        void out(uint32_t w, uint32_t flag) override {
            if (flag) { row_read(w, true); return; }
            const uint32_t row = c.row_of(w);
            if (w >= c.p.n_witnesses || row == NONE) { c.finding(std::string(who) + " writes witness " + std::to_string(w) + ", which has no row, in " + c.launch_name(c.cur)); return; }
            c.write(RK_W, row, w, who);
        }
        void mem_r(uint32_t first, uint32_t n) override { for (uint32_t i = 0; i < n; i++) c.read(RK_MEM, first + i, NONE, who); }
        void mem_w(uint32_t first, uint32_t n) override { for (uint32_t i = 0; i < n; i++) c.write(RK_MEM, first + i, NONE, who); }
        void byte_in(uint32_t w) override {
            const uint32_t pl = c.p.byte_plane_of.empty() || w >= c.p.byte_plane_of.size() ? NONE : c.p.byte_plane_of[w];
            if (pl == NONE) { row_read(w, true); return; }
            c.read(RK_BYTE_PLANE, pl, w, who);
        }
        void dig(uint32_t w, uint32_t unscale_row) override {
            Res *r = row_read(w, false);
            if (w >= c.p.n_witnesses) return;
            if (unscale_row != c.p.unscale_index[w]) c.finding("REPRESENTATION: a digest leaf multiplies witness " + std::to_string(w) + " by the wrong 1 / scale");
            if (r && unscale_row == NONE && !r->canon) c.finding("REPRESENTATION: a digest leaf reads witness " + std::to_string(w) + " as it is but " + c.launch_name(r->w_launch) + " stored a relaxed row");
        }
        void leaf(uint32_t row) override { c.write(RK_LEAF, row, NONE, who); }
    };

    void walk_wave_program(uint32_t gate_index) {
        const std::vector<uint32_t> &gs = p.gate_stream;
        size_t pos = p.gate_offset[gate_index];
        uint32_t local_kb = GATE_K_CANON, local_witness = NONE;
        bool host = true;
        for (;;) {
            if (pos + 6 > gs.size()) { finding("gate record runs past the stream"); return; }
            const uint32_t w0 = gs[pos], kind = w0 & 0xff, opcode = gs[pos + 1], w5 = gs[pos + 5];
            const uint32_t np_mac = (w0 >> 8) & 0xff, nl_mac = (w0 >> 16) & 0xff, n_mac = np_mac + nl_mac;
            const uint32_t np_pos = w5 & 0xff, np_neg = (w5 >> 8) & 0xff, nl_pos = (w5 >> 16) & 0xff, nl_neg = w5 >> 24;
            const uint32_t sub_k = (w0 >> GATE_SUBK_SHIFT) & 3u;
            rep.n_records++;
            char who[64];
            snprintf(who, sizeof who, "gate of opcode %u", opcode);
            if (opcode >= p.n_opcodes || p.prog[p.prog_offset[opcode]] != PK_ARITH) { finding(std::string(who) + " is not an Arithmetic opcode"); return; }
            const uint32_t out_w = out_of[opcode].empty() ? NONE : out_of[opcode][0];
            std::vector<uint32_t> cand;
            {
                const size_t e = p.prog_offset[opcode] + 2;
                const uint32_t n_mul = p.prog[e], n_lin = p.prog[e + 1];
                size_t t = e + 3;
                for (uint32_t i = 0; i < n_mul; i++, t += 3) {
                    if (p.prog[t] == COEF_ZERO) continue;
                    const uint32_t l = p.prog[t + 1], r = p.prog[t + 2];
                    if (l == out_w || r == out_w) continue;
                    cand.push_back(l); cand.push_back(r);
                }
                for (uint32_t i = 0; i < n_lin; i++, t += 3)
                    if (p.prog[t] != COEF_ZERO && p.prog[t + 2] != out_w) cand.push_back(p.prog[t + 2]);
                std::sort(cand.begin(), cand.end());
                cand.erase(std::unique(cand.begin(), cand.end()), cand.end());
            }
            std::vector<uint8_t> matched(cand.size(), 0);
            bool uses_local = false;
            auto operand = [&](uint32_t row) -> uint32_t {
                if (row == GATE_LOCAL) {
                    uses_local = true;
                    if (host) finding(std::string(who) + " reads the wave's forwarded value but heads its wave program");
                    return local_kb;
                }
                uint32_t want = NONE;
// ... 123 lines not shown
                prev_end = std::max(prev_end, off + words);
            }
        }
        if (scratch && prev_end) { cur_prog = 0x7FFFFFFFu; write(RK_SCRATCH, cls, NONE, "class scratch"); }
    }

    ScheduleReport run(uint32_t drop_wait) {
        replay();
        std::array<uint32_t, N_SCHED_STREAMS> zero{};
        std::array<std::array<uint32_t, N_SCHED_STREAMS>, N_SCHED_STREAMS> clock{};
        uint32_t seq[N_SCHED_STREAMS] = {0, 0, 0, 0, 0, 0};
        const uint32_t n_events = 2 * p.n_levels + 1 + 4 * p.n_levels;
        std::vector<std::array<uint32_t, N_SCHED_STREAMS>> ev(n_events, zero);
        std::vector<uint8_t> ev_set(n_events, 0);
        auto new_launch = [&](uint8_t stream, uint8_t op, uint32_t level, uint32_t step) {
            Launch l;
            l.stream = stream; l.op = op; l.level = level; l.step = step;
            l.seq = ++seq[stream];
            clock[stream][stream] = l.seq;
            l.clock = clock[stream];
            l.clock[stream] = l.seq - 1;
            launches.push_back(l);
            cur = (int)launches.size() - 1;
            cur_prog = 0;
            rep.n_launches++;
        };
        new_launch(SS_MAIN, 0xFE, 0, 0);
        for (uint32_t w : p.initial_ids) {
            const uint32_t row = row_of(w);
            if (row == NONE) { finding("initial witness " + std::to_string(w) + " has no row"); continue; }
            write(RK_W, row, w, "import");
            if (!p.byte_plane_of.empty() && p.byte_plane_of[w] != NONE) write(RK_BYTE_PLANE, p.byte_plane_of[w], w, "import");
        }
        int reset_launch = -1;
        uint32_t wait_index = 0;
        for (size_t si = 0; si < sch.steps.size(); si++) {
            const SchedStep &st = sch.steps[si];
            if (st.stream >= N_SCHED_STREAMS) { finding("step on an unknown stream"); continue; }
            if (st.kind == SK_RECORD) {
                if (st.event >= n_events) { finding("record of an event outside the handle's pools"); continue; }
                ev[st.event] = clock[st.stream];
                ev_set[st.event] = 1;
                continue;
            }
            if (st.kind == SK_WAIT) {
                rep.n_waits++;
                if (wait_index++ == drop_wait) {
                    bool implied = st.event < n_events && ev_set[st.event];
                    for (int q = 0; q < N_SCHED_STREAMS && implied; q++) implied = ev[st.event][q] <= clock[st.stream][q];
                    char buf[160];
                    snprintf(buf, sizeof buf, "(mutation: wait #%u dropped -- step %zu, stream %u waits for event %u%s)\n", drop_wait, si, st.stream, st.event,
                             implied ? "; everything behind that event was already ordered before this stream: a redundant wait" : "");
                    rep.text += buf;
                    continue;
                }
                if (st.event >= n_events || !ev_set[st.event]) { finding("step " + std::to_string(si) + " waits for an event that has not been recorded in this solve (a no-op on the device)"); continue; }
                for (int q = 0; q < N_SCHED_STREAMS; q++) clock[st.stream][q] = std::max(clock[st.stream][q], ev[st.event][q]);
                continue;
            }
            new_launch(st.stream, st.op, st.level, (uint32_t)si);
            if (st.op == SO_EVENT_RESET) { reset_launch = cur; continue; }
            if (reset_launch < 0 || !hb(reset_launch, cur)) finding("EVENT WORDS: " + launch_name(cur) + " may flag instances before the event words are reset");
            switch (st.op) {
            case SO_GATES: case SO_GATES_LIGHT:
                if ((uint64_t)st.first + st.count > p.gate_offset.size()) { finding("gate launch runs past the gate list"); break; }
                for (uint32_t g = st.first; g < st.first + st.count; g++) { cur_prog = g; walk_wave_program(g); }
// ... 38 lines not shown
```

acvm_amd/csrc/tuning.cpp:

```cpp
#include "tuning.hpp"
#include <cstdlib>
#include <cstring>
#include <mutex>
#include <string>

namespace acvm {
namespace {

struct Key { const char *name; int64_t Tuning::*field; };
const Key KEYS[] = {
    {"scale", &Tuning::scale}, {"relax", &Tuning::relax}, {"pedersen_bundle", &Tuning::pedersen_bundle}, {"pedersen_bundle_waves", &Tuning::pedersen_bundle_waves}, {"pairs", &Tuning::pairs}, {"chains", &Tuning::chains}, {"max_tails", &Tuning::max_tails},
    {"inv_epoch", &Tuning::inv_epoch}, {"inv_latency", &Tuning::inv_latency}, {"inv_chunk", &Tuning::inv_chunk}, {"inv_share", &Tuning::inv_share}, {"byte_plane", &Tuning::byte_plane}, {"heavy_epoch", &Tuning::heavy_epoch}, {"heavy_latency", &Tuning::heavy_latency},
    {"pedersen_latency", &Tuning::pedersen_latency}, {"pedersen_epoch", &Tuning::pedersen_epoch}, {"digest_epoch", &Tuning::digest_epoch}, {"range_fuse", &Tuning::range_fuse},
    {"range_merge", &Tuning::range_merge}, {"hash_chain", &Tuning::hash_chain}, {"brillig_inline", &Tuning::brillig_inline}, {"sl_lane", &Tuning::sl_lane},
    {"pedersen_waves", &Tuning::pedersen_waves}, {"pedersen_prio", &Tuning::pedersen_prio}, {"light_fuse", &Tuning::light_fuse}, {"plan_validate", &Tuning::plan_validate}, {"brillig_mem_cells", &Tuning::brillig_mem_cells}, {"overlap", &Tuning::overlap}, {"heavy_streams", &Tuning::heavy_streams}, {"heavy_only_streams", &Tuning::heavy_only_streams},
    {"fc_relevel", &Tuning::fc_relevel}, {"exact_async", &Tuning::exact_async}, {"brillig_steps_log2", &Tuning::brillig_steps_log2},
    {"brillig_steps_max_log2", &Tuning::brillig_steps_max_log2}, {"brillig_call_depth", &Tuning::brillig_call_depth},
    {"brillig_call_depth_max", &Tuning::brillig_call_depth_max}, {"brillig_mem_max_log2", &Tuning::brillig_mem_max_log2},
    {"pedersen_window_bits", &Tuning::pedersen_window_bits}, {"win16", &Tuning::win16}, {"tables_keep", &Tuning::tables_keep},
};
constexpr unsigned N_KEYS = sizeof KEYS / sizeof KEYS[0];

Tuning g_tuning;
std::once_flag g_env_once;

void read_env() {
    const char *e = getenv("ACVM_TUNING");
    if (!e) return;
    std::string s(e);
    size_t at = 0;
    while (at < s.size()) {
        size_t end = s.find(',', at);
        if (end == std::string::npos) end = s.size();
        const std::string item = s.substr(at, end - at);
        const size_t eq = item.find('=');
        if (eq != std::string::npos) {
            const std::string k = item.substr(0, eq);
            for (const Key &key : KEYS)
                if (k == key.name) g_tuning.*key.field = strtoll(item.c_str() + eq + 1, nullptr, 10);
        }
        at = end + 1;
    }
}

}
// ... 24 lines not shown
```

acvm_amd/csrc/tuning.hpp:

```cpp
#pragma once
#include <stdint.h>

namespace acvm {

struct Tuning {
    int64_t scale = 1;
    int64_t relax = 1;
    int64_t pairs = 1;
    int64_t chains = 1;
    int64_t max_tails = 5;
    int64_t inv_epoch = 4;
    int64_t byte_plane = 1;
    int64_t inv_chunk = 128;
    int64_t inv_share = 4;
    int64_t inv_latency = 1;
    int64_t heavy_epoch = 1;
    int64_t heavy_latency = 0;
    int64_t pedersen_latency = 4;
    int64_t pedersen_epoch = 8;
    int64_t digest_epoch = 8;
    int64_t range_fuse = 1;
    int64_t range_merge = 1;
    int64_t hash_chain = 1;
    int64_t brillig_inline = 1;
    int64_t sl_lane = 0;
    int64_t pedersen_waves = 0;
    int64_t pedersen_bundle = 1;
    int64_t pedersen_bundle_waves = 2048;
    int64_t pedersen_prio = 1;
    int64_t light_fuse = 1;
    int64_t plan_validate = 0;
    int64_t brillig_mem_cells = 0;
    int64_t overlap = 1;
    int64_t heavy_streams = 1;
    int64_t heavy_only_streams = 1;
    int64_t fc_relevel = -1;
    int64_t exact_async = 1;
    int64_t brillig_steps_log2 = 22, brillig_steps_max_log2 = 26;
    int64_t brillig_call_depth = 64, brillig_call_depth_max = 1 << 16;
    int64_t brillig_mem_max_log2 = 22;
    int64_t pedersen_window_bits = 24;
    int64_t win16 = 1;
    int64_t tables_keep = 1;
};

Tuning &tuning();
bool tuning_set(const char *key, int64_t value);
// ... 5 lines not shown
```

include/acvm_amd.h:

```cpp
#ifndef ACVM_AMD_H
#define ACVM_AMD_H
#include <stddef.h>
#include <stdint.h>

#ifdef __cplusplus
extern "C" {
#endif

#define ACVM_AMD_ABI_VERSION 6

enum {
    ACVM_OK = 0,
    ACVM_E_INVALID = -1,
    ACVM_E_MALFORMED = -2,
    ACVM_E_UNSUPPORTED = -3,
    ACVM_E_DEVICE = -4,
    ACVM_E_STATE = -5,
    ACVM_E_NOMEM = -6
};

enum { ACVM_STATUS_SOLVED = 0, ACVM_STATUS_IN_PROGRESS = 1, ACVM_STATUS_FAILURE = 2, ACVM_STATUS_REQUIRES_FOREIGN_CALL = 3 };

enum {
    ACVM_ERR_NONE = 0,
// ... 61 lines not shown
    uint32_t n_inverse_slots;
    uint32_t n_scaled_witnesses;
    uint32_t n_arith_launches;
    uint32_t n_table_rows;
    uint32_t n_digest_segments;
    uint32_t n_brillig_inlined;
    uint32_t n_brillig_retries;
    uint32_t n_hash_chained;
    uint32_t n_gate_out_asis, n_gate_out_weak, n_gate_out_canon, max_gate_bound;
    uint32_t n_byte_planes, n_byte_plane_reads;
    uint32_t n_stream_launches[6], n_stream_waits;
} acvm_stats_t;

const char *acvm_last_error(void);
int acvm_abi_version(void);
int acvm_device_count(void);
int acvm_set_device(int device);
int acvm_device_synchronize(void);
int acvm_device_arch(char *out, size_t out_len);
long long acvm_device_release_tables(int device);

int acvm_tuning_set(const char *key, long long value);
int acvm_tuning_get(const char *key, long long *value);
const char *acvm_tuning_key(unsigned index);

int acvm_selftest(uint32_t n, uint64_t seed);

int acvm_debug_grumpkin(uint32_t what, uint32_t param, const uint8_t *in_be32, uint32_t n_in, uint8_t *out_be64);
int acvm_debug_table_info(uint32_t table, uint64_t *n_entries, int *built);
int acvm_debug_table_read(uint32_t table, const uint64_t *entries, uint32_t n, uint32_t *out_words16);
int acvm_debug_batch_tables(const acvm_batch_t *b, uint32_t *mask);
int acvm_debug_secp(uint32_t curve, uint32_t what, const uint8_t *in_be32, uint32_t n_items, uint8_t *out_be32);
int acvm_debug_fr(uint32_t what, const uint32_t *in, uint32_t n_items, const uint32_t *uniform18, uint32_t *out);
int acvm_debug_inverse_batch(const uint32_t *den, uint32_t n_jobs, uint32_t B, uint32_t inv_chunk, const uint32_t *slot_of, uint32_t *inv_out,
                             uint32_t *event_out, uint32_t *device_count, uint32_t *host_count);
int acvm_debug_inverse_batch_shared(const uint32_t *den, uint32_t n_jobs, uint32_t B, uint32_t inv_chunk, uint32_t inv_share, const uint32_t *slot_of,
                                    uint32_t *inv_out, uint32_t *event_out, uint32_t *device_count, uint32_t *host_count);
int acvm_debug_select(const uint8_t *status, uint32_t n, uint32_t select_mask, uint32_t *out_list, uint32_t *n_selected);

int acvm_debug_modmul_rate(uint32_t iters, uint32_t waves_per_simd, double *modmul_per_s, uint64_t *n_modmul);
int acvm_debug_secp_rate(uint32_t curve, uint32_t iters, uint32_t waves_per_simd, double *products_per_s, uint64_t *n_products);
int acvm_debug_stream_rate(size_t bytes, double *gb_per_s);

acvm_circuit_t *acvm_circuit_from_bytes(const uint8_t *bytes, size_t len);
void acvm_circuit_free(acvm_circuit_t *c);
uint32_t acvm_circuit_num_opcodes(const acvm_circuit_t *c);
uint32_t acvm_circuit_num_witnesses(const acvm_circuit_t *c);
int acvm_circuit_opcode_kinds(const acvm_circuit_t *c, uint32_t first, uint32_t n, uint32_t *kinds );
int acvm_circuit_plan_stats(const acvm_circuit_t *c, const uint32_t *initial_ids, uint32_t n_initial, acvm_stats_t *out);
uint64_t acvm_circuit_plans_built(const acvm_circuit_t *c);
int acvm_circuit_plan_stats_ex(const acvm_circuit_t *c, const uint32_t *initial_ids, uint32_t n_initial, uint32_t flags, const uint32_t *keep_ids,
                               uint32_t n_keep, acvm_stats_t *out);

int acvm_circuit_check_schedule(const acvm_circuit_t *c, const uint32_t *initial_ids, uint32_t n_initial, uint32_t flags, const uint32_t *keep_ids, uint32_t n_keep,
                                uint32_t n_instances, uint32_t drop_wait, uint64_t *counts , char *report, size_t report_len);
int acvm_debug_plan_fingerprint(const acvm_circuit_t *c, const uint32_t *initial_ids, uint32_t n_initial, uint32_t flags, const uint32_t *keep_ids,
                                uint32_t n_keep, uint64_t *out, uint32_t cap);
acvm_batch_t *acvm_batch_new(const acvm_circuit_t *c, const acvm_bb_solver_t *solver, uint32_t n_instances,
                             const uint32_t *initial_ids, uint32_t n_initial);
#define ACVM_BATCH_FOLD_DIGEST 1u
#define ACVM_BATCH_REUSE_SLOTS 2u
acvm_batch_t *acvm_batch_new_ex(const acvm_circuit_t *c, const acvm_bb_solver_t *solver, uint32_t n_instances, const uint32_t *initial_ids,
                                uint32_t n_initial, uint32_t flags, const uint32_t *keep_ids, uint32_t n_keep);
void acvm_batch_free(acvm_batch_t *b);
int acvm_batch_set_initial_witness(acvm_batch_t *b, const uint8_t *values_be32);
int acvm_batch_set_initial_witness_device(acvm_batch_t *b, const void *d_values_be32);
// ... 293 lines not shown
```

Baseline: 6.104 million witnesses/s.

## Precompute per-coefficient linear tables to fuse Montgomery reduction into linear-term accumulation

Adds a precomputed 81-word table for each linear-only gate coefficient. The table folds the coefficient together with the reduction constants, so the gate kernel can accumulate linear terms through a column-wise multiply-add with a fused Montgomery step instead of the generic dot-product-then-reduce path. Tables and per-program offsets are built in the plan, uploaded to the device, passed to the arith kernels and checked by the schedule validator. In exchange, each term reads 81 words of table memory (scalar loads) rather than a 9-word coefficient, and the plan grows in size.

```diff
diff --git a/acvm_amd/__init__.py b/acvm_amd/__init__.py
--- a/acvm_amd/__init__.py
+++ b/acvm_amd/__init__.py
@@ -45,6 +45,7 @@
     "acvm_node_set_foreign_call_handler", "acvm_node_foreign_stats",
     "acvm_batch_import_device_records", "acvm_batch_set_initial_witness_records", "acvm_node_solve_records",
     "acvm_batch_export_device_records", "acvm_batch_witness_records",
+    "acvm_debug_lin_add", "acvm_debug_lin_plan",
 ]
 
 
@@ -408,6 +409,9 @@
     L.acvm_circuit_plans_built.restype = C.c_uint64
     L.acvm_circuit_plans_built.argtypes = [C.c_void_p]
     L.acvm_circuit_check_schedule.argtypes = [C.c_void_p, C.c_void_p, C.c_uint32, C.c_uint32, C.c_void_p, C.c_uint32, C.c_uint32, C.c_uint32, C.POINTER(C.c_uint64), C.c_char_p, C.c_size_t]
+    if hasattr(L, "acvm_debug_lin_plan"):
+        L.acvm_debug_lin_plan.argtypes = [C.c_void_p, C.c_void_p, C.c_uint32, C.c_uint32, C.c_void_p, C.c_uint32, C.c_uint32, C.c_uint32, C.POINTER(C.c_uint64), C.c_char_p, C.c_size_t]
+        L.acvm_debug_lin_add.argtypes = [C.c_void_p, C.c_void_p, C.c_void_p, C.c_void_p, C.c_uint32, C.c_void_p, C.c_void_p]
     L.acvm_batch_new.restype = C.c_void_p
     L.acvm_batch_new.argtypes = [C.c_void_p, C.c_void_p, C.c_uint32, C.c_void_p, C.c_uint32]
     L.acvm_batch_new_ex.restype = C.c_void_p
@@ -726,6 +730,20 @@
     return out
 
 
+def debug_lin_add(n_terms, coef, rows, h):
+    import numpy as np
+    nt = np.ascontiguousarray(n_terms, dtype=np.uint32).reshape(-1)
+    r = np.ascontiguousarray(rows, dtype=np.uint32)
+    n = r.shape[0]
+    n_groups = (n + 63) // 64
+    cf = np.ascontiguousarray(coef, dtype=np.uint32)
+    hh = np.ascontiguousarray(h, dtype=np.uint32)
+    assert nt.shape == (n_groups,) and cf.shape == (n_groups, 2, 8) and r.shape == (n, 2, 8) and hh.shape == (n, 9)
+    tables, out = np.zeros((n_groups, 2, 81), dtype=np.uint32), np.zeros((n, 9), dtype=np.uint32)
+    _check(lib().acvm_debug_lin_add(nt.ctypes.data, cf.ctypes.data, r.ctypes.data, hh.ctypes.data, n, tables.ctypes.data, out.ctypes.data))
+    return tables, out
+
+
 def debug_inverse_batch(den, inv_chunk, slot_of=None, inv_share=None):
     import numpy as np
     d = np.ascontiguousarray(den, dtype=np.uint32)
@@ -832,6 +850,19 @@
         _check(rc)
         return {"ok": rc == 0, "n_launches": counts[0], "n_waits": counts[1], "n_accesses": counts[2], "n_records": counts[3], "n_findings": counts[4],
                 "report": text.value.decode()}
+
+    def lin_plan(self, initial_ids, n_instances=4096, fold_digest=False, reuse_slots=False, keep=(), mutation=0) -> dict:
+        ids = list(initial_ids)
+        arr = (C.c_uint32 * max(len(ids), 1))(*ids)
+        keep = list(keep)
+        karr = (C.c_uint32 * max(len(keep), 1))(*keep)
+        counts = (C.c_uint64 * 8)()
+        text = C.create_string_buffer(1 << 14)
+        rc = lib().acvm_debug_lin_plan(self._h, arr, len(ids), (1 if fold_digest else 0) | (2 if reuse_slots else 0), karr, len(keep), n_instances, mutation,
+                                       counts, text, len(text))
+        _check(rc)
+        return {"ok": rc == 0, "n_wave_programs": counts[0], "n_programs_with_tables": counts[1], "n_gate_records": counts[2], "n_lin_records": counts[3],
+                "n_lin_terms": counts[4], "n_findings": counts[5], "report": text.value.decode()}
 
     def plan_fingerprint(self, initial_ids, fold_digest=False, reuse_slots=False, keep=(), host_solver=False) -> list:
         ids = list(initial_ids)
diff --git a/acvm_amd/csrc/batch.cpp b/acvm_amd/csrc/batch.cpp
--- a/acvm_amd/csrc/batch.cpp
+++ b/acvm_amd/csrc/batch.cpp
@@ -10,6 +10,7 @@
 #include <string>
 #include <vector>
 #include "batch_internal.hpp"
+#include "gate_record.hpp"
 
 static thread_local std::string g_last_error;
 int set_err(int code, const std::string &msg) {
@@ -217,7 +218,7 @@
 
 static size_t plan_bytes(const Plan &p) {
     size_t words = p.gate_stream.size() + p.gate_offset.size() + p.prog.size() + p.prog_offset.size() + p.prog_scratch.size() + p.bytecode.size() + p.slot_of.size() + p.kbound.size() +
-                   p.unscale_index.size() + p.scaled_ids.size() + p.producer.size() + p.byte_plane_of.size() + p.dyn_offset.size();
+                   p.unscale_index.size() + p.scaled_ids.size() + p.producer.size() + p.byte_plane_of.size() + p.dyn_offset.size() + p.lin_tables.size() + p.lin_offset.size();
     for (int k = 0; k < (int)N_CLS; k++) words += 2 * p.cls_offset[k].size();
     return words * 4 + (p.constants.size() + p.unscale.size()) * sizeof(FrH);
 }
@@ -277,6 +278,48 @@
     const LevelSchedule sched = level_schedule(*sp, lay);
     const ScheduleReport rep = check_level_schedule(*sp, lay, sched, drop_wait);
     if (counts) { counts[0] = rep.n_launches; counts[1] = rep.n_waits; counts[2] = rep.n_accesses; counts[3] = rep.n_records; counts[4] = rep.n_findings; }
+    if (report && report_len) snprintf(report, report_len, "%s", rep.text.c_str());
+    return rep.ok ? 0 : 1;
+} ABI_CATCH
+
+int acvm_debug_lin_plan(const acvm_circuit_t *c, const uint32_t *initial_ids, uint32_t n_initial, uint32_t flags, const uint32_t *keep_ids, uint32_t n_keep,
+                        uint32_t n_instances, uint32_t mutation, uint64_t *counts, char *report, size_t report_len) try {
+    if (!c || (n_initial && !initial_ids) || (n_keep && !keep_ids)) return set_err(ACVM_E_INVALID, "null argument");
+    PlanOpts opts;
+    opts.fold_digest = (flags & (ACVM_BATCH_FOLD_DIGEST | ACVM_BATCH_REUSE_SLOTS)) != 0;
+    opts.reuse_slots = (flags & ACVM_BATCH_REUSE_SLOTS) != 0;
+    opts.host_blackbox = (flags & 0x100u) != 0;
+    opts.keep.assign(keep_ids, keep_ids + n_keep);
+    const std::shared_ptr<const Plan> sp = plan_for(c, initial_ids, n_initial, opts);
+    if (!sp->unsupported.empty()) return set_err(ACVM_E_UNSUPPORTED, sp->unsupported);
+    Plan p = *sp;
+    const size_t n_tables = p.lin_tables.size() / GATE_LIN_TABLE_WORDS;
+    if (mutation == 1) {
+        size_t other = 0;
+        for (size_t t = 1; t < n_tables && !other; t++)
+            if (memcmp(&p.lin_tables[0], &p.lin_tables[t * GATE_LIN_TABLE_WORDS], GATE_LIN_TABLE_WORDS * 4) != 0) other = t;
+        if (!other) return set_err(ACVM_E_INVALID, "the plan has no two tables that differ");
+        std::swap_ranges(p.lin_tables.begin(), p.lin_tables.begin() + GATE_LIN_TABLE_WORDS, p.lin_tables.begin() + other * GATE_LIN_TABLE_WORDS);
+    } else if (mutation == 2) {
+        size_t q = 0;
+        while (q < p.lin_offset.size() && p.lin_offset[q] == GATE_LIN_NONE) q++;
+        if (q == p.lin_offset.size()) return set_err(ACVM_E_INVALID, "the plan has no table");
+        p.lin_offset[q]++;
+    } else if (mutation) return set_err(ACVM_E_INVALID, "no such mutation");
+    const LaunchLayout lay = layout_launches(p, ((uint64_t)n_instances + 63) / 64 * 64);
+    const LevelSchedule sched = level_schedule(p, lay);
+    const ScheduleReport rep = check_level_schedule(p, lay, sched, 0xFFFFFFFFu);
+    if (counts) {
+        uint64_t with = 0, records = 0;
+        for (size_t q = 0; q < p.gate_offset.size(); q++) {
+            with += q < p.lin_offset.size() && p.lin_offset[q] != GATE_LIN_NONE;
+            for (size_t pos = p.gate_offset[q];; pos += gate_record_words(GATE_WORDS(&p.gate_stream[pos]))) {
+                records++;
+                if (!(p.gate_stream[pos] & GATE_TAIL_FLAG)) break;
+            }
+        }
+        counts[0] = p.gate_offset.size(); counts[1] = with; counts[2] = records; counts[3] = p.n_lin_records; counts[4] = p.n_lin_terms; counts[5] = rep.n_findings;
+    }
     if (report && report_len) snprintf(report, report_len, "%s", rep.text.c_str());
     return rep.ok ? 0 : 1;
 } ABI_CATCH
@@ -341,6 +384,8 @@
     HIPCHK(hipMalloc((void **)&b->d_W, w_bytes ? w_bytes : 16));
     if (int rc = upload(&b->d_gate_stream, p.gate_stream)) return rc;
     if (int rc = upload(&b->d_gate_offset, p.gate_offset)) return rc;
+    if (int rc = upload(&b->d_lin_tables, p.lin_tables)) return rc;
+    if (int rc = upload(&b->d_lin_offset, p.lin_offset)) return rc;
     std::vector<uint32_t> consts(p.constants.size() * 8);
     for (size_t i = 0; i < p.constants.size(); i++) {
         const FrH d = frh::to_device_form(p.constants[i]);
diff --git a/acvm_amd/csrc/batch.hpp b/acvm_amd/csrc/batch.hpp
--- a/acvm_amd/csrc/batch.hpp
+++ b/acvm_amd/csrc/batch.hpp
@@ -78,6 +78,7 @@
     hipStream_t stream = nullptr;
     uint4 *d_W = nullptr, *d_Mem = nullptr;
     uint32_t *d_gate_stream = nullptr, *d_gate_offset = nullptr, *d_consts = nullptr;
+    uint32_t *d_lin_tables = nullptr, *d_lin_offset = nullptr;
     uint32_t *d_prog = nullptr, *d_prog_offset = nullptr, *d_bytecode = nullptr, *d_init_ids = nullptr, *d_producer = nullptr;
     uint32_t *d_dyn_offset = nullptr, *d_slow_start = nullptr;
     uint8_t *d_prog_class = nullptr;
@@ -217,7 +218,7 @@
         hipSetDevice(device);
         for (void *p : {(void *)d_W, (void *)d_Mem, (void *)d_gate_stream, (void *)d_gate_offset, (void *)d_consts, (void *)d_prog,
                         (void *)d_prog_offset, (void *)d_bytecode, (void *)d_init_ids, (void *)d_producer, (void *)d_dyn_offset,
-                        (void *)d_slow_start, (void *)d_event_base, (void *)d_slow_ids, (void *)d_assigned, (void *)d_slow_res})
+                        (void *)d_slow_start, (void *)d_lin_tables, (void *)d_lin_offset, (void *)d_event_base, (void *)d_slow_ids, (void *)d_assigned, (void *)d_slow_res})
             if (p) hipFree(p);
         if (h_flag_count) hipHostFree(h_flag_count);
         for (int k = 0; k < (int)N_CLS; k++)
diff --git a/acvm_amd/csrc/batch_schedule.cpp b/acvm_amd/csrc/batch_schedule.cpp
--- a/acvm_amd/csrc/batch_schedule.cpp
+++ b/acvm_amd/csrc/batch_schedule.cpp
@@ -45,11 +45,12 @@
             b->events_fresh = false;
             break;
         case SO_GATES:
-            launch_arith_level(s, b->d_W, b->Bp, b->B, b->d_gate_stream, b->d_gate_offset + st.first, st.count, b->d_consts, b->d_event, b->d_inv);
+            launch_arith_level(s, b->d_W, b->Bp, b->B, b->d_gate_stream, b->d_gate_offset + st.first, st.count, b->d_consts, b->d_event, b->d_inv, b->d_lin_tables,
+                               b->d_lin_offset + st.first);
             break;
         case SO_GATES_LIGHT:
             launch_arith_light_level(s, b->d_W, b->Bp, b->B, b->d_gate_stream, b->d_gate_offset + st.first, st.count, b->d_inv, b->dp,
-                                     b->d_cls_offset[CLS_LIGHT] + st.first2, st.count2, b->d_event);
+                                     b->d_cls_offset[CLS_LIGHT] + st.first2, st.count2, b->d_event, b->d_lin_tables, b->d_lin_offset + st.first);
             break;
         case SO_LIGHT: launch_light_level(s, b->d_W, b->Bp, b->B, b->dp, off, st.count, b->d_event); break;
         case SO_LIGHT_SL: launch_light_sl_level(s, b->d_W, b->Bp, b->B, b->dp, off, st.count, b->d_event); break;
diff --git a/acvm_amd/csrc/fr_device.hpp b/acvm_amd/csrc/fr_device.hpp
--- a/acvm_amd/csrc/fr_device.hpp
+++ b/acvm_amd/csrc/fr_device.hpp
@@ -346,6 +346,55 @@
 FR_HD __forceinline__ Fr29 fr29_dot(const Fr29 (&a)[N], const Fr29 (&b)[N]) { return fr29_dot_impl<N, false>(a, b, nullptr); }
 template <int N>
 FR_HD __forceinline__ Fr29 fr29_dot_add(const Fr29 (&a)[N], const Fr29 (&b)[N], const Fr29 &h) { return fr29_dot_impl<N, true>(a, b, &h); }
+
+template <int N, class T>
+FR_HD __forceinline__ Fr29 fr29_lin_add(T tab, const Fr29 (&x)[N], const Fr29 &h) {
+    static_assert(N == 1 || N == 2, "column accumulator budget");
+    constexpr uint32_t M = 0x1fffffffu;
+    uint64_t acc = 0;
+    uint32_t m[2];
+    Fr29 r;
+    uint32_t c[9 * N], nx[9];
+#pragma unroll
+    for (int i = 0; i < 9; i++) c[i] = tab[i];
+#pragma unroll
+    for (int k = 0; k < 9; k++) {
+        T next = tab;
+#if defined(__HIP_DEVICE_COMPILE__)
+        asm volatile("" : "+s"(next), "+v"(acc));
+#endif
+        if (k < 8) {
+#pragma unroll
+            for (int i = 0; i < 9; i++) nx[i] = next[9 * (k + 1) + i];
+        }
+        if (N == 2) {
+#pragma unroll
+            for (int i = 0; i < 9; i++) c[9 + i] = next[81 + 9 * k + i];
+        }
+#pragma unroll
+        for (int t = 0; t < N; t++)
+#pragma unroll
+            for (int i = 0; i < 9; i++) acc += (uint64_t)x[t].v[i] * c[9 * t + i];
+#pragma unroll
+        for (int i = 0; i < 9; i++) c[i] = nx[i];
+        if (k >= 1) acc += (uint64_t)m[0] * fr_p29(k);
+        if (k >= 2) acc += (uint64_t)m[1] * fr_p29(k - 1);
+        if (k < 2) {
+            const uint32_t lo = (uint32_t)acc;
+            m[k] = (((lo & 1u) << 28) - lo) & M;
+            acc += ((uint64_t)m[k] << 28) + m[k];
+        } else {
+            acc += h.v[k - 2];
+            r.v[k - 2] = (uint32_t)acc & M;
+        }
+        acc >>= 29;
+    }
+    acc += (uint64_t)m[1] * fr_p29(8) + h.v[7];
+    r.v[7] = (uint32_t)acc & M;
+    acc >>= 29;
+    r.v[8] = (uint32_t)acc + h.v[8];
+    return r;
+}
 
 #if defined(__HIP_DEVICE_COMPILE__) && !defined(FR_NO_ASM_BLOCKS)
 #define FR_ASM_BLOCKS 1
diff --git a/acvm_amd/csrc/gate_eval.hpp b/acvm_amd/csrc/gate_eval.hpp
--- a/acvm_amd/csrc/gate_eval.hpp
+++ b/acvm_amd/csrc/gate_eval.hpp
@@ -52,7 +52,7 @@
 }
 
 template <class L>
-FR_HD __forceinline__ Fr29 gate_eval(const L &ld, GateWords g, const Fr29 &local) {
+FR_HD __forceinline__ Fr29 gate_eval(L &ld, GateWords g, const Fr29 &local) {
     const uint32_t w0 = g[0], w5 = g[5], qc = g[3], kind = w0 & 0xff;
     const uint32_t np_mac = (w0 >> 8) & 0xff, nl_mac = (w0 >> 16) & 0xff, n_mac = np_mac + nl_mac;
     const uint32_t np_pos = w5 & 0xff, np_neg = (w5 >> 8) & 0xff, nl_pos = (w5 >> 16) & 0xff, nl_neg = w5 >> 24;
@@ -94,9 +94,20 @@
         h = fr29_dot_add_b<2, 2u>(l, m, h);
         GATE_AFTER_REDUCTION();
     }
+    const bool lin = ld.has_lin() && gate_lin_terms(w0, w5) != 0;
     for (; im < n_mac; im += 2) {
         GateWords c0 = gate_mac_entry(t0, np_mac, im);
-        if (n_mac - im == 1) {
+        if (lin) {
+            if (n_mac - im == 1) {
+                const Fr29 l[1] = {gate_operand(ld, c0[8], local)};
+                h = fr29_lin_add<1>(ld.lin, l, h);
+                ld.lin += GATE_LIN_TABLE_WORDS;
+            } else {
+                const Fr29 l[2] = {gate_operand(ld, c0[8], local), gate_operand(ld, gate_mac_entry(t0, np_mac, im + 1)[8], local)};
+                h = fr29_lin_add<2>(ld.lin, l, h);
+                ld.lin += 2 * GATE_LIN_TABLE_WORDS;
+            }
+        } else if (n_mac - im == 1) {
             const Fr29 l[1] = {gate_mac_operand(ld, c0, im < np_mac, local)}, m[1] = {gate_coef29(c0)};
             h = fr29_dot_add_b<1, 1u>(l, m, h);
         } else {
diff --git a/acvm_amd/csrc/gate_record.hpp b/acvm_amd/csrc/gate_record.hpp
--- a/acvm_amd/csrc/gate_record.hpp
+++ b/acvm_amd/csrc/gate_record.hpp
@@ -37,6 +37,12 @@
     return (uint32_t)(((uint64_t)ka * kb * 1549u + ((1ull << 26) - 1)) >> 26);
 }
 
+static constexpr uint32_t GATE_LIN_TABLE_WORDS = 81;
+static constexpr uint32_t GATE_LIN_NONE = 0xFFFFFFFFu;
+GATE_HD inline uint32_t gate_lin_terms(uint32_t w0, uint32_t w5) {
+    return ((w0 >> 8) & 0xff) == 0 && (w5 & 0xff) == 0 ? (w0 >> 16) & 0xff : 0u;
+}
+
 GATE_HD inline uint32_t gate_record_words(GateWords g) {
     const uint32_t w0 = g[0], w5 = g[5];
     return 6u + 10u * ((w0 >> 8) & 0xff) + 9u * ((w0 >> 16) & 0xff) + 2u * ((w5 & 0xff) + ((w5 >> 8) & 0xff)) + ((w5 >> 16) & 0xff) + (w5 >> 24);
diff --git a/acvm_amd/csrc/kernels.hip b/acvm_amd/csrc/kernels.hip
--- a/acvm_amd/csrc/kernels.hip
+++ b/acvm_amd/csrc/kernels.hip
@@ -287,8 +287,9 @@
 #endif
 __global__ void __launch_bounds__(ARITH_BLOCK) __attribute__((amdgpu_waves_per_eu(ARITH_WAVES_MIN, 8)))
 arith_level_kernel(uint4 *__restrict__ W, uint64_t Bp, uint32_t B, const uint32_t *__restrict__ gate_stream, const uint32_t *__restrict__ gate_offset,
-                   const uint32_t *__restrict__ consts, uint32_t *__restrict__ event, const uint4 *__restrict__ Inv) {
-    arith_level_body(W, Bp, B, gate_stream, gate_offset, consts, event, Inv, blockIdx.y);
+                   const uint32_t *__restrict__ consts, uint32_t *__restrict__ event, const uint4 *__restrict__ Inv, const uint32_t *__restrict__ lin_tables,
+                   const uint32_t *__restrict__ lin_offset) {
+    arith_level_body(W, Bp, B, gate_stream, gate_offset, consts, event, Inv, lin_tables, lin_offset, blockIdx.y);
 }
 
 struct InverseDevicePolicy {
@@ -433,6 +434,32 @@
     hipLaunchKernelGGL(fr_probe_kernel, dim3((n_items + 63) / 64), dim3(64), 0, s, what, in, n_items, fr_probe_words_in(what), fr_probe_words_out(what), un, out);
 }
 
+__global__ void __launch_bounds__(64) lin_add_probe_kernel(const uint32_t *__restrict__ n_terms, const uint32_t *__restrict__ tables, const uint32_t *__restrict__ rows,
+                                                           const uint32_t *__restrict__ hs, uint32_t n_items, uint32_t *__restrict__ out) {
+    const uint32_t t = blockIdx.x * 64 + threadIdx.x;
+    if (t >= n_items) return;
+    GateWords tab = GATE_WORDS(tables) + (uint64_t)blockIdx.x * 2 * GATE_LIN_TABLE_WORDS;
+    Fr a, b;
+    Fr29 h, r;
+#pragma unroll
+    for (int i = 0; i < 8; i++) { a.v[i] = rows[(size_t)t * 16 + i]; b.v[i] = rows[(size_t)t * 16 + 8 + i]; }
+#pragma unroll
+    for (int i = 0; i < 9; i++) h.v[i] = hs[(size_t)t * 9 + i];
+    if (n_terms[blockIdx.x] == 1) {
+        const Fr29 x[1] = {fr29_from(a)};
+        r = fr29_lin_add<1>(tab, x, h);
+    } else {
+        const Fr29 x[2] = {fr29_from(a), fr29_from(b)};
+        r = fr29_lin_add<2>(tab, x, h);
+    }
+#pragma unroll
+    for (int i = 0; i < 9; i++) out[(size_t)t * 9 + i] = r.v[i];
+}
+void launch_lin_add_probe(hipStream_t s, const uint32_t *n_terms, const uint32_t *tables, const uint32_t *rows, const uint32_t *hs, uint32_t n_items, uint32_t *out) {
+    if (!n_items) return;
+    hipLaunchKernelGGL(lin_add_probe_kernel, dim3((n_items + 63) / 64), dim3(64), 0, s, n_terms, tables, rows, hs, n_items, out);
+}
+
 __global__ void __launch_bounds__(256) modmul_rate_kernel(uint32_t *__restrict__ out, uint32_t seed, uint32_t iters) {
     Fr29 a, b;
 #pragma unroll
@@ -591,10 +618,11 @@
                        u.consts, producer, start_opcode);
 }
 void launch_arith_level(hipStream_t s, uint4 *W, uint64_t Bp, uint32_t B, const uint32_t *gate_stream, const uint32_t *gate_offset,
-                        uint32_t n_gates, const uint32_t *consts, uint32_t *event, const uint4 *inv) {
+                        uint32_t n_gates, const uint32_t *consts, uint32_t *event, const uint4 *inv, const uint32_t *lin_tables, const uint32_t *lin_offset) {
     for (uint32_t done = 0; done < n_gates;) {
         uint32_t n = n_gates - done > 65535u ? 65535u : n_gates - done;
-        hipLaunchKernelGGL(arith_level_kernel, dim3((B + ARITH_BLOCK - 1) / ARITH_BLOCK, n), dim3(ARITH_BLOCK), 0, s, W, Bp, B, gate_stream, gate_offset + done, consts, event, inv);
+        hipLaunchKernelGGL(arith_level_kernel, dim3((B + ARITH_BLOCK - 1) / ARITH_BLOCK, n), dim3(ARITH_BLOCK), 0, s, W, Bp, B, gate_stream, gate_offset + done, consts, event, inv, lin_tables,
+                           lin_offset + done);
         done += n;
     }
 }
diff --git a/acvm_amd/csrc/kernels.hpp b/acvm_amd/csrc/kernels.hpp
--- a/acvm_amd/csrc/kernels.hpp
+++ b/acvm_amd/csrc/kernels.hpp
@@ -153,16 +153,18 @@
 void launch_unscale_slow(hipStream_t s, uint4 *W, uint64_t Bp, const uint32_t *slow_ids, uint32_t n_slow, const Unscale &u, const uint32_t *producer,
                          const uint32_t *start_opcode);
 void launch_arith_level(hipStream_t s, uint4 *W, uint64_t Bp, uint32_t B, const uint32_t *gate_stream, const uint32_t *gate_offset,
-                        uint32_t n_gates, const uint32_t *consts, uint32_t *event, const uint4 *inv);
+                        uint32_t n_gates, const uint32_t *consts, uint32_t *event, const uint4 *inv, const uint32_t *lin_tables, const uint32_t *lin_offset);
 void launch_inverse_batch(hipStream_t s, const uint4 *W, uint4 *inv, uint64_t Bp, uint32_t B, const uint32_t *gate_stream,
                           const uint32_t *job_offset, uint32_t n_jobs, uint32_t *event, uint32_t inv_chunk, uint32_t inv_share);
 inline uint32_t inverse_share_clamp(int64_t v) { return v >= 8 ? 8u : v >= 4 ? 4u : v >= 2 ? 2u : 1u; }
 void launch_arith_light_level(hipStream_t s, uint4 *W, uint64_t Bp, uint32_t B, const uint32_t *gate_stream, const uint32_t *gate_offset, uint32_t n_gates,
-                              const uint4 *inv, const DeviceProgram &dp, const uint32_t *light_offsets, uint32_t n_light, uint32_t *event);
+                              const uint4 *inv, const DeviceProgram &dp, const uint32_t *light_offsets, uint32_t n_light, uint32_t *event, const uint32_t *lin_tables,
+                              const uint32_t *lin_offset);
 void launch_modmul_rate(hipStream_t s, uint32_t *out, uint32_t blocks, uint32_t iters);
 void launch_secp_rate(hipStream_t s, uint32_t curve, uint32_t *out, uint32_t blocks, uint32_t iters);
 void launch_stream_rate(hipStream_t s, const uint4 *a, const uint4 *b, uint4 *out, uint64_t n);
 void launch_fr_selftest(hipStream_t s, uint64_t seed, uint32_t n, uint32_t *mismatches);
+void launch_lin_add_probe(hipStream_t s, const uint32_t *n_terms, const uint32_t *tables, const uint32_t *rows, const uint32_t *hs, uint32_t n_items, uint32_t *out);
 uint32_t fr_probe_words(uint32_t what, bool out);
 void launch_fr_probe(hipStream_t s, uint32_t what, const uint32_t *in, uint32_t n_items, const uint32_t *uniform18, uint32_t *out);
 void launch_fill_u32(hipStream_t s, uint32_t *p, uint32_t v, uint64_t n);
diff --git a/acvm_amd/csrc/kernels_ops.hip b/acvm_amd/csrc/kernels_ops.hip
--- a/acvm_amd/csrc/kernels_ops.hip
+++ b/acvm_amd/csrc/kernels_ops.hip
@@ -134,9 +134,10 @@
 __global__ void __launch_bounds__(256) __attribute__((amdgpu_waves_per_eu(6, 8)))
 arith_light_level_kernel(uint4 *__restrict__ W, uint64_t Bp, uint32_t B, const uint32_t *__restrict__ gate_stream, const uint32_t *__restrict__ gate_offset,
                          const uint32_t *__restrict__ consts, uint32_t *__restrict__ event, const uint4 *__restrict__ Inv, uint32_t n_light,
-                         const uint32_t *__restrict__ light_offsets, const uint32_t *__restrict__ prog, const uint32_t *__restrict__ slot_of, uint4 *Mem) {
+                         const uint32_t *__restrict__ light_offsets, const uint32_t *__restrict__ prog, const uint32_t *__restrict__ slot_of, uint4 *Mem,
+                         const uint32_t *__restrict__ lin_tables, const uint32_t *__restrict__ lin_offset) {
     if (blockIdx.y >= n_light) {
-        arith_level_body(W, Bp, B, gate_stream, gate_offset, consts, event, Inv, blockIdx.y - n_light);
+        arith_level_body(W, Bp, B, gate_stream, gate_offset, consts, event, Inv, lin_tables, lin_offset, blockIdx.y - n_light);
         return;
     }
     const uint64_t j = (uint64_t)blockIdx.x * 256 + threadIdx.x;
@@ -147,10 +148,11 @@
     if (r.err) flag_instance(event, j, rec[0] == K_RANGE_MULTI ? r.aux0 : rec[1]);
 }
 void launch_arith_light_level(hipStream_t s, uint4 *W, uint64_t Bp, uint32_t B, const uint32_t *gate_stream, const uint32_t *gate_offset, uint32_t n_gates,
-                              const uint4 *inv, const DeviceProgram &dp, const uint32_t *light_offsets, uint32_t n_light, uint32_t *event) {
+                              const uint4 *inv, const DeviceProgram &dp, const uint32_t *light_offsets, uint32_t n_light, uint32_t *event, const uint32_t *lin_tables,
+                              const uint32_t *lin_offset) {
     if (!B || !(n_gates + n_light)) return;
     hipLaunchKernelGGL(arith_light_level_kernel, dim3((B + 255) / 256, n_gates + n_light), dim3(256), 0, s, W, Bp, B, gate_stream, gate_offset, dp.consts, event, inv,
-                       n_light, light_offsets, dp.prog, dp.slot_of, dp.Mem);
+                       n_light, light_offsets, dp.prog, dp.slot_of, dp.Mem, lin_tables, lin_offset);
 }
 void launch_light_sl_level(hipStream_t s, uint4 *W, uint64_t Bp, uint32_t B, const DeviceProgram &dp, const uint32_t *offsets, uint32_t n,
                            uint32_t *event) {
diff --git a/acvm_amd/csrc/lin_table.hpp b/acvm_amd/csrc/lin_table.hpp
--- /dev/null
+++ b/acvm_amd/csrc/lin_table.hpp
@@ -0,0 +1,24 @@
+#pragma once
+#include "fr_host.hpp"
+#include "gate_record.hpp"
+
+namespace acvm {
+
+inline void lin_table_of(const uint32_t *coef, uint32_t *out) {
+    FrH d;
+    for (int i = 0; i < 4; i++) d.l[i] = coef[2 * i] | (uint64_t)coef[2 * i + 1] << 32;
+    FrH t = frh::mul(frh::from_device_form(d), frh::from_u64(1ull << 58));
+    const FrH step = frh::from_u64(1ull << 29);
+    for (int i = 0; i < 9; i++, t = frh::mul(t, step)) {
+        uint64_t v[4];
+        frh::to_canonical(t, v);
+        for (int k = 0; k < 9; k++) {
+            const int bit = 29 * k, w = bit >> 6, sh = bit & 63;
+            uint64_t limb = v[w] >> sh;
+            if (sh > 35 && w + 1 < 4) limb |= v[w + 1] << (64 - sh);
+            out[9 * k + i] = (uint32_t)limb & 0x1fffffffu;
+        }
+    }
+}
+
+}
diff --git a/acvm_amd/csrc/ops_common.hpp b/acvm_amd/csrc/ops_common.hpp
--- a/acvm_amd/csrc/ops_common.hpp
+++ b/acvm_amd/csrc/ops_common.hpp
@@ -66,6 +66,8 @@
     const uint4 *__restrict__ Inv;
     const uint32_t *__restrict__ consts;
     uint64_t Bp, j;
+    GateWords lin;
+    __device__ __forceinline__ bool has_lin() const { return lin != GATE_WORDS(nullptr); }
     __device__ __forceinline__ Fr29 load(uint32_t slot) const {
 #ifdef GATE_EXP_NO_LOADS
         Fr29 r;
@@ -83,11 +85,13 @@
 };
 __device__ __forceinline__ void arith_level_body(uint4 *__restrict__ W, uint64_t Bp, uint32_t B, const uint32_t *__restrict__ gate_stream,
                                                  const uint32_t *__restrict__ gate_offset, const uint32_t *__restrict__ consts,
-                                                 uint32_t *__restrict__ event, const uint4 *__restrict__ Inv, uint32_t gate_index) {
+                                                 uint32_t *__restrict__ event, const uint4 *__restrict__ Inv, const uint32_t *__restrict__ lin_tables,
+                                                 const uint32_t *__restrict__ lin_offset, uint32_t gate_index) {
     const uint64_t j = (uint64_t)blockIdx.x * blockDim.x + threadIdx.x;
     if (j >= B) return;
     GateWords g = GATE_WORDS(gate_stream) + gate_offset[gate_index];
-    const GateDeviceLoader ld{W, Inv, consts, Bp, j};
+    const uint32_t lin_at = lin_offset[gate_index];
+    GateDeviceLoader ld{W, Inv, consts, Bp, j, lin_at != GATE_LIN_NONE ? GATE_WORDS(lin_tables) + (uint64_t)lin_at * GATE_LIN_TABLE_WORDS : GATE_WORDS(nullptr)};
     Fr29 local = fr29_from(fr_zero());
     bool host = true;
     for (;;) {
diff --git a/acvm_amd/csrc/plan.cpp b/acvm_amd/csrc/plan.cpp
--- a/acvm_amd/csrc/plan.cpp
+++ b/acvm_amd/csrc/plan.cpp
@@ -1,5 +1,6 @@
 #include "plan.hpp"
 #include "gate_record.hpp"
+#include "lin_table.hpp"
 #include "tuning.hpp"
 #include "scratch_layout.hpp"
 #include <algorithm>
@@ -290,6 +291,30 @@
                 for (uint32_t r = lo; r < hi; r++)
                     if ((pg[p.cls_offset[k][r]] == PK_BRILLIG_SL) == (pass == 1)) recs.push_back({p.cls_offset[k][r], p.cls_scratch[k][r]});
             for (uint32_t r = lo; r < hi; r++) { p.cls_offset[k][r] = recs[r - lo].first; p.cls_scratch[k][r] = recs[r - lo].second; }
+        }
+    }
+}
+
+void build_lin_tables(Plan &p) {
+    p.lin_tables.clear();
+    p.lin_offset.assign(p.gate_offset.size(), GATE_LIN_NONE);
+    p.n_lin_records = p.n_lin_terms = 0;
+    if (!p.tune.lin_table) return;
+    const std::vector<uint32_t> &gs = p.gate_stream;
+    for (size_t q = 0; q < p.gate_offset.size(); q++) {
+        for (size_t pos = p.gate_offset[q];;) {
+            const uint32_t w0 = gs[pos], n_terms = gate_lin_terms(w0, gs[pos + 5]);
+            if (n_terms) {
+                if (p.lin_offset[q] == GATE_LIN_NONE) p.lin_offset[q] = p.n_lin_terms;
+                p.n_lin_records++;
+                for (uint32_t i = 0; i < n_terms; i++) {
+                    p.lin_tables.resize(p.lin_tables.size() + GATE_LIN_TABLE_WORDS);
+                    lin_table_of(&gs[pos + 6 + 9 * (size_t)i], &p.lin_tables[(size_t)p.n_lin_terms * GATE_LIN_TABLE_WORDS]);
+                    p.n_lin_terms++;
+                }
+            }
+            if (!(w0 & GATE_TAIL_FLAG)) break;
+            pos += gate_record_words(GATE_WORDS(&gs[pos]));
         }
     }
 }
@@ -1768,6 +1793,7 @@
     b.lay_out();
     if (v) b.check_layout();
     order_level_records(b.p);
+    build_lin_tables(b.p);
     return b.finish();
 }
 
diff --git a/acvm_amd/csrc/plan.hpp b/acvm_amd/csrc/plan.hpp
--- a/acvm_amd/csrc/plan.hpp
+++ b/acvm_amd/csrc/plan.hpp
@@ -36,6 +36,9 @@
     uint32_t n_byte_planes = 0, n_byte_plane_reads = 0;
     std::vector<uint32_t> gate_stream;
     std::vector<uint32_t> gate_offset;
+    std::vector<uint32_t> lin_tables;
+    std::vector<uint32_t> lin_offset;
+    uint32_t n_lin_records = 0, n_lin_terms = 0;
     std::vector<uint32_t> level_start;
     std::vector<uint32_t> dyn_offset;
     std::vector<uint32_t> dyn_level_start;
diff --git a/acvm_amd/csrc/probes.cpp b/acvm_amd/csrc/probes.cpp
--- a/acvm_amd/csrc/probes.cpp
+++ b/acvm_amd/csrc/probes.cpp
@@ -10,6 +10,7 @@
 #include <string>
 #include <vector>
 #include "batch_internal.hpp"
+#include "lin_table.hpp"
 
 int acvm_selftest(uint32_t n, uint64_t seed) {
     uint32_t *d = nullptr, h = 0;
@@ -262,6 +263,41 @@
     return rc;
 } ABI_CATCH
 
+int acvm_debug_lin_add(const uint32_t *n_terms, const uint32_t *coef, const uint32_t *rows, const uint32_t *h, uint32_t n_items, uint32_t *tables_out, uint32_t *out) try {
+    if (!n_items) return 0;
+    if (!n_terms || !coef || !rows || !h || !out) return set_err(ACVM_E_INVALID, "null argument");
+    const size_t n_groups = ((size_t)n_items + 63) / 64;
+    std::vector<uint32_t> tables(n_groups * 2 * GATE_LIN_TABLE_WORDS, 0);
+    for (size_t g = 0; g < n_groups; g++) {
+        if (n_terms[g] != 1 && n_terms[g] != 2) return set_err(ACVM_E_INVALID, "a group has one or two terms");
+        for (uint32_t t = 0; t < n_terms[g]; t++) {
+            uint64_t c[4];
+            for (int i = 0; i < 4; i++) c[i] = coef[g * 16 + t * 8 + 2 * i] | (uint64_t)coef[g * 16 + t * 8 + 2 * i + 1] << 32;
+            if (frh::geq_p(c)) return set_err(ACVM_E_INVALID, "a coefficient is not canonical");
+            const FrH d = frh::to_device_form(frh::from_canonical(c));
+            uint32_t inline_words[8];
+            for (int i = 0; i < 4; i++) { inline_words[2 * i] = (uint32_t)d.l[i]; inline_words[2 * i + 1] = (uint32_t)(d.l[i] >> 32); }
+            lin_table_of(inline_words, &tables[(g * 2 + t) * GATE_LIN_TABLE_WORDS]);
+        }
+    }
+    if (tables_out) memcpy(tables_out, tables.data(), tables.size() * 4);
+    const size_t bytes[5] = {n_groups * 4, tables.size() * 4, (size_t)n_items * 16 * 4, (size_t)n_items * 9 * 4, (size_t)n_items * 9 * 4};
+    const void *src[4] = {n_terms, tables.data(), rows, h};
+    uint32_t *d[5] = {nullptr, nullptr, nullptr, nullptr, nullptr};
+    int rc = 0;
+    auto step = [&](hipError_t e, const char *what_) { if (!rc && e != hipSuccess) rc = set_err(ACVM_E_DEVICE, std::string(what_) + ": " + hipGetErrorString(e)); };
+    for (int k = 0; k < 5; k++) step(hipMalloc((void **)&d[k], bytes[k]), "hipMalloc");
+    for (int k = 0; k < 4 && !rc; k++) step(hipMemcpy(d[k], src[k], bytes[k], hipMemcpyHostToDevice), "hipMemcpy");
+    if (!rc) step(hipMemset(d[4], 0, bytes[4]), "hipMemset");
+    if (!rc) launch_lin_add_probe(nullptr, d[0], d[1], d[2], d[3], n_items, d[4]);
+    step(hipGetLastError(), "lin_add_probe_kernel");
+    step(hipDeviceSynchronize(), "hipDeviceSynchronize");
+    if (!rc) step(hipMemcpy(out, d[4], bytes[4], hipMemcpyDeviceToHost), "hipMemcpy");
+    for (int k = 0; k < 5; k++)
+        if (d[k]) hipFree(d[k]);
+    return rc;
+} ABI_CATCH
+
 static int debug_inverse_batch(const uint32_t *den, uint32_t n_jobs, uint32_t B, uint32_t inv_chunk, uint32_t inv_share, const uint32_t *slot_of, uint32_t *inv_out,
                                uint32_t *event_out, uint32_t *device_count, uint32_t *host_count) {
     if (!den || !n_jobs || !B || !inv_out || !event_out || !device_count || !host_count) return set_err(ACVM_E_INVALID, "bad argument");
diff --git a/acvm_amd/csrc/schedule_check.cpp b/acvm_amd/csrc/schedule_check.cpp
--- a/acvm_amd/csrc/schedule_check.cpp
+++ b/acvm_amd/csrc/schedule_check.cpp
@@ -1,4 +1,5 @@
 #include "gate_record.hpp"
+#include "lin_table.hpp"
 #include "schedule.hpp"
 #include <array>
 #include <cstdio>
@@ -371,9 +372,24 @@
         size_t pos = p.gate_offset[gate_index];
         uint32_t local_kb = GATE_K_CANON, local_witness = NONE;
         bool host = true;
+        uint64_t lin_at = gate_index < p.lin_offset.size() ? p.lin_offset[gate_index] : GATE_LIN_NONE;
+        const bool has_lin = lin_at != GATE_LIN_NONE;
         for (;;) {
             if (pos + 6 > gs.size()) { finding("gate record runs past the stream"); return; }
             const uint32_t w0 = gs[pos], kind = w0 & 0xff, opcode = gs[pos + 1], w5 = gs[pos + 5];
+            if (const uint32_t n_terms = gate_lin_terms(w0, w5)) {
+                if (pos + 6 + 9 * (size_t)n_terms > gs.size()) { finding("gate record runs past the stream"); return; }
+                if (!has_lin) {
+                    if (p.tune.lin_table) finding("LINEAR TABLES: gate of opcode " + std::to_string(opcode) + " qualifies for the table form but its wave program (" + std::to_string(gate_index) + ") lists no table");
+                } else {
+                    for (uint32_t i = 0; i < n_terms; i++, lin_at++) {
+                        if ((lin_at + 1) * GATE_LIN_TABLE_WORDS > p.lin_tables.size()) { finding("LINEAR TABLES: gate of opcode " + std::to_string(opcode) + ", term " + std::to_string(i) + ": the cursor (table " + std::to_string(lin_at) + ") runs past the tables"); break; }
+                        uint32_t want[GATE_LIN_TABLE_WORDS];
+                        lin_table_of(&gs[pos + 6 + 9 * (size_t)i], want);
+                        if (memcmp(want, &p.lin_tables[lin_at * GATE_LIN_TABLE_WORDS], sizeof want) != 0) finding("LINEAR TABLES: gate of opcode " + std::to_string(opcode) + ", term " + std::to_string(i) + ": table " + std::to_string(lin_at) + " at the kernel's cursor is not the table of the record's coefficient (wave program " + std::to_string(gate_index) + ")");
+                    }
+                }
+            }
             const uint32_t np_mac = (w0 >> 8) & 0xff, nl_mac = (w0 >> 16) & 0xff, n_mac = np_mac + nl_mac;
             const uint32_t np_pos = w5 & 0xff, np_neg = (w5 >> 8) & 0xff, nl_pos = (w5 >> 16) & 0xff, nl_neg = w5 >> 24;
             const uint32_t sub_k = (w0 >> GATE_SUBK_SHIFT) & 3u;
@@ -563,6 +579,7 @@
             write(RK_W, row, w, "import");
             if (!p.byte_plane_of.empty() && p.byte_plane_of[w] != NONE) write(RK_BYTE_PLANE, p.byte_plane_of[w], w, "import");
         }
+        if (p.lin_offset.size() != p.gate_offset.size()) finding("LINEAR TABLES: " + std::to_string(p.lin_offset.size()) + " table offsets for " + std::to_string(p.gate_offset.size()) + " wave programs (the gate kernel reads one per program)");
         int reset_launch = -1;
         uint32_t wait_index = 0;
         for (size_t si = 0; si < sch.steps.size(); si++) {
diff --git a/acvm_amd/csrc/tuning.cpp b/acvm_amd/csrc/tuning.cpp
--- a/acvm_amd/csrc/tuning.cpp
+++ b/acvm_amd/csrc/tuning.cpp
@@ -10,7 +10,7 @@
 struct Key { const char *name; int64_t Tuning::*field; };
 const Key KEYS[] = {
     {"scale", &Tuning::scale}, {"relax", &Tuning::relax}, {"pedersen_bundle", &Tuning::pedersen_bundle}, {"pedersen_bundle_waves", &Tuning::pedersen_bundle_waves}, {"pairs", &Tuning::pairs}, {"chains", &Tuning::chains}, {"max_tails", &Tuning::max_tails},
-    {"inv_epoch", &Tuning::inv_epoch}, {"inv_latency", &Tuning::inv_latency}, {"inv_chunk", &Tuning::inv_chunk}, {"inv_share", &Tuning::inv_share}, {"byte_plane", &Tuning::byte_plane}, {"heavy_epoch", &Tuning::heavy_epoch}, {"heavy_latency", &Tuning::heavy_latency},
+    {"inv_epoch", &Tuning::inv_epoch}, {"inv_latency", &Tuning::inv_latency}, {"inv_chunk", &Tuning::inv_chunk}, {"inv_share", &Tuning::inv_share}, {"lin_table", &Tuning::lin_table},{"byte_plane", &Tuning::byte_plane}, {"heavy_epoch", &Tuning::heavy_epoch}, {"heavy_latency", &Tuning::heavy_latency},
     {"pedersen_latency", &Tuning::pedersen_latency}, {"pedersen_epoch", &Tuning::pedersen_epoch}, {"digest_epoch", &Tuning::digest_epoch}, {"range_fuse", &Tuning::range_fuse},
     {"range_merge", &Tuning::range_merge}, {"hash_chain", &Tuning::hash_chain}, {"brillig_inline", &Tuning::brillig_inline}, {"sl_lane", &Tuning::sl_lane},
     {"pedersen_waves", &Tuning::pedersen_waves}, {"pedersen_prio", &Tuning::pedersen_prio}, {"light_fuse", &Tuning::light_fuse}, {"plan_validate", &Tuning::plan_validate}, {"brillig_mem_cells", &Tuning::brillig_mem_cells}, {"overlap", &Tuning::overlap}, {"heavy_streams", &Tuning::heavy_streams}, {"heavy_only_streams", &Tuning::heavy_only_streams},
diff --git a/acvm_amd/csrc/tuning.hpp b/acvm_amd/csrc/tuning.hpp
--- a/acvm_amd/csrc/tuning.hpp
+++ b/acvm_amd/csrc/tuning.hpp
@@ -13,6 +13,7 @@
     int64_t byte_plane = 1;
     int64_t inv_chunk = 128;
     int64_t inv_share = 4;
+    int64_t lin_table = 1;
     int64_t inv_latency = 1;
     int64_t heavy_epoch = 1;
     int64_t heavy_latency = 0;
diff --git a/include/acvm_amd.h b/include/acvm_amd.h
--- a/include/acvm_amd.h
+++ b/include/acvm_amd.h
@@ -117,6 +117,9 @@
 int acvm_debug_batch_tables(const acvm_batch_t *b, uint32_t *mask);
 int acvm_debug_secp(uint32_t curve, uint32_t what, const uint8_t *in_be32, uint32_t n_items, uint8_t *out_be32);
 int acvm_debug_fr(uint32_t what, const uint32_t *in, uint32_t n_items, const uint32_t *uniform18, uint32_t *out);
+int acvm_debug_lin_add(const uint32_t *n_terms, const uint32_t *coef, const uint32_t *rows, const uint32_t *h, uint32_t n_items, uint32_t *tables_out, uint32_t *out);
+int acvm_debug_lin_plan(const acvm_circuit_t *c, const uint32_t *initial_ids, uint32_t n_initial, uint32_t flags, const uint32_t *keep_ids, uint32_t n_keep,
+                        uint32_t n_instances, uint32_t mutation, uint64_t *counts, char *report, size_t report_len);
 int acvm_debug_inverse_batch(const uint32_t *den, uint32_t n_jobs, uint32_t B, uint32_t inv_chunk, const uint32_t *slot_of, uint32_t *inv_out,
                              uint32_t *event_out, uint32_t *device_count, uint32_t *host_count);
 int acvm_debug_inverse_batch_shared(const uint32_t *den, uint32_t n_jobs, uint32_t B, uint32_t inv_chunk, uint32_t inv_share, const uint32_t *slot_of,
```

Measured after the change: 6.238 million witnesses/s, median of 6. 2.2% higher.
